# genlm/genlm-backend

Hardware: AMD Instinct MI355X
Metric: particles/sec + logprob-kernel HBM GB/s (% of 8 TB/s), 1024 particles gpt2 (higher is better)
Workload: dtype f32

## Files before the change

### genlm-backend_amd/_lib.py

```python
import ctypes as C
import os

_HERE = os.path.dirname(os.path.abspath(__file__))
LIB_PATH = os.path.join(_HERE, "libglb_hip.so")

ABI_VERSION = 9
GLB_OK, GLB_EINVAL, GLB_EUNSUPPORTED, GLB_EHIP, GLB_ENOSPC = 0, 1, 2, 3, 4
F32, BF16, F16 = 0, 1, 2
MASK_NONE, MASK_BITS, MASK_F32, MASK_PREPARED = 0, 1, 2, 3
RNG_NONE, RNG_PHILOX, RNG_NOISE = 0, 1, 2
STEP_HW_EXP = 1
GEMM_BIAS, GEMM_BIAS_GELU_TANH = 0, 1
GEMM_FORM_LARGE, GEMM_FORM_SMALL = 1, 2


class GlbError(RuntimeError):
    def __init__(self, code, msg):
        super().__init__(f"glb error {code}: {msg}")
        self.code = code


class StepArgs(C.Structure):
    _fields_ = [
        ("struct_size", C.c_uint32),
# ... 310 lines not shown
class FsaProductArgs(C.Structure):
    _fields_ = [
        ("struct_size", C.c_uint32),
        ("op", C.c_int32),
        ("n_a", C.c_int32), ("n_b", C.c_int32), ("start_a", C.c_int32), ("start_b", C.c_int32),
        ("delta_a", C.c_void_p), ("delta_b", C.c_void_p),
        ("accepting_a", C.c_void_p), ("accepting_b", C.c_void_p),
        ("live_a", C.c_void_p), ("live_b", C.c_void_p),
        ("arc_a", C.c_void_p), ("final_a", C.c_void_p),
        ("arc_b", C.c_void_p), ("final_b", C.c_void_p),
        ("max_states", C.c_int32),
        ("n_states", C.c_int32),
        ("table", C.c_void_p), ("table_slots", C.c_int64),
        ("pairs", C.c_void_p), ("delta_out", C.c_void_p), ("accepting_out", C.c_void_p),
        ("arc_out", C.c_void_p), ("final_out", C.c_void_p),
        ("live", C.c_void_p), ("counts", C.c_void_p), ("status", C.c_void_p),
        ("rounds", C.c_int32), ("restart", C.c_int32),
    ]


NFA_STATUS = 16
NFA_CLOSURE_STATUS = 8
NFA_MAX_IMPORTANT = 4096
NFA_MAX_STATES = 1 << 22


class NfaArgs(C.Structure):
    _fields_ = [
        ("struct_size", C.c_uint32),
        ("n_states", C.c_int32), ("start", C.c_int32),
        ("n_important", C.c_int32), ("n_words", C.c_int32),
        ("n_arcs", C.c_int32), ("n_eps", C.c_int32), ("n_groups", C.c_int32),
        ("eps_off", C.c_void_p), ("eps_to", C.c_void_p), ("bit_of", C.c_void_p),
        ("arc_off", C.c_void_p), ("arc_dst", C.c_void_p), ("arc_bytes", C.c_void_p), ("accepting_mask", C.c_void_p),
        ("group_of", C.c_void_p), ("group_lo", C.c_void_p),
        ("eclose", C.c_void_p),
        ("hash_mask", C.c_uint64),
        ("max_states", C.c_int32), ("chunk", C.c_int32),
        ("table", C.c_void_p), ("table_slots", C.c_int64),
        ("cand", C.c_void_p), ("sets", C.c_void_p),
        ("delta_out", C.c_void_p), ("accepting_out", C.c_void_p), ("counts", C.c_void_p), ("status", C.c_void_p),
        ("rounds", C.c_int32), ("restart", C.c_int32),
    ]


LAZY_STATUS = 8
LAZY_OVERFLOW, LAZY_BUG = 1, 2


class LazyArgs(C.Structure):
    _fields_ = [
        ("struct_size", C.c_uint32),
        ("dfa", DfaArgs),
        ("n_nfa_states", C.c_int32), ("nfa_start", C.c_int32),
        ("n_important", C.c_int32), ("n_words", C.c_int32),
        ("n_arcs", C.c_int32),
        ("max_states", C.c_int32),
        ("arc_off", C.c_void_p), ("arc_dst", C.c_void_p), ("arc_bytes", C.c_void_p), ("accepting_mask", C.c_void_p),
        ("eclose", C.c_void_p),
        ("hash_mask", C.c_uint64),
        ("table", C.c_void_p), ("table_slots", C.c_int64),
        ("cand", C.c_void_p), ("counts", C.c_void_p), ("cand_rows", C.c_int64),
        ("sets", C.c_void_p), ("accepting_out", C.c_void_p), ("status", C.c_void_p),
        ("row_state", C.c_void_p), ("row_stamp", C.c_void_p), ("claimants", C.c_void_p), ("victims", C.c_void_p),
        ("ecounters", C.c_void_p), ("epoch", C.c_void_p),
        ("force_wave", C.c_int32),
    ]


PDA_MAX_DEPTH = 504
PDA_STATUS = 8
PDA_OVERFLOW, PDA_BUG = 1, 2
PDA_MAX_SYMBOLS, PDA_POP = 126, 127


class PdaArgs(C.Structure):
    _fields_ = [
        ("struct_size", C.c_uint32),
        ("dfa", DfaArgs),
        ("n_pda_states", C.c_int32), ("n_symbols", C.c_int32), ("start", C.c_int32),
        ("max_depth", C.c_int32), ("n_words", C.c_int32), ("max_states", C.c_int32),
        ("delta", C.c_void_p), ("accepting", C.c_void_p),
        ("hash_mask", C.c_uint64),
        ("table", C.c_void_p), ("table_slots", C.c_int64),
        ("cand", C.c_void_p), ("counts", C.c_void_p), ("cand_rows", C.c_int64),
        ("configs", C.c_void_p), ("accepting_out", C.c_void_p), ("status", C.c_void_p),
        ("row_state", C.c_void_p), ("row_stamp", C.c_void_p), ("claimants", C.c_void_p), ("victims", C.c_void_p),
        ("ecounters", C.c_void_p), ("epoch", C.c_void_p),
        ("max_token_bytes", C.c_int32),
    ]


CONJ_MAX_PARTS = 8
CONJ_STATUS = 8
CONJ_OVERFLOW, CONJ_BUG = 1, 2


class ConjArgs(C.Structure):
    _fields_ = [
        ("struct_size", C.c_uint32),
        ("dfa", DfaArgs),
        ("n_parts", C.c_int32), ("n_words", C.c_int32), ("max_states", C.c_int32),
        ("part_start", C.c_int32 * CONJ_MAX_PARTS),
        ("hash_mask", C.c_uint64),
        ("table", C.c_void_p), ("table_slots", C.c_int64),
        ("tuples", C.c_void_p), ("status", C.c_void_p),
        ("counts", C.c_void_p), ("cand_rows", C.c_int64),
        ("part_states", C.c_void_p), ("part_ld", C.c_int64),
        ("claim_states", C.c_void_p), ("rep", C.c_void_p),
        ("part_rows", C.c_void_p * CONJ_MAX_PARTS), ("part_bank", C.c_void_p * CONJ_MAX_PARTS),
        ("part_bank_ld", C.c_int64 * CONJ_MAX_PARTS), ("part_capacity", C.c_int64 * CONJ_MAX_PARTS),
        ("part_weighted", C.c_int32 * CONJ_MAX_PARTS),
        ("wbank", C.c_void_p), ("wbank_ld", C.c_int64),
        ("row_state", C.c_void_p), ("row_stamp", C.c_void_p), ("claimants", C.c_void_p), ("victims", C.c_void_p),
        ("ecounters", C.c_void_p), ("epoch", C.c_void_p),
    ]


class ImportanceArgs(C.Structure):
    _fields_ = [
        ("struct_size", C.c_uint32),
        ("target", C.c_void_p), ("target_dtype", C.c_int32), ("ld_p", C.c_int64),
        ("proposal", C.c_void_p), ("proposal_dtype", C.c_int32), ("ld_q", C.c_int64),
        ("n_rows", C.c_int64), ("vocab", C.c_int64),
        ("proposal_scale", C.c_float),
        ("n_particles", C.c_int64), ("row_of", C.c_void_p),
        ("mask_kind", C.c_int32), ("mask", C.c_void_p), ("mask_ld", C.c_int64), ("n_masks", C.c_int64),
        ("mask_id", C.c_void_p), ("row_mask_id", C.c_void_p),
        ("seed", C.c_uint64), ("offset", C.c_uint64), ("particle_base", C.c_int64),
        ("out_token", C.c_void_p), ("out_dlogw", C.c_void_p), ("out_lse_target", C.c_void_p),
        ("out_logZ_proposal", C.c_void_p),
        ("workspace", C.c_void_p), ("workspace_bytes", C.c_size_t),
    ]


IMPORTANCE_CHUNK = 4096
IMPORTANCE_RECORD_BYTES = 64


class ScoreArgs(C.Structure):
    _fields_ = [
        ("struct_size", C.c_uint32),
        ("logits", C.c_void_p), ("dtype", C.c_int32),
        ("n_rows", C.c_int64), ("vocab", C.c_int64), ("ld", C.c_int64),
        ("logit_scale", C.c_float),
        ("token", C.c_void_p),
        ("mask_kind", C.c_int32), ("mask", C.c_void_p), ("mask_ld", C.c_int64), ("n_masks", C.c_int64),
        ("row_mask_id", C.c_void_p),
        ("out_logp", C.c_void_p), ("out_lse", C.c_void_p), ("out_logZ", C.c_void_p), ("out_logp_masked", C.c_void_p),
        ("seq_start", C.c_void_p), ("n_seq", C.c_int64),
        ("out_seq_logp", C.c_void_p), ("out_seq_logZ", C.c_void_p), ("out_seq_logp_masked", C.c_void_p),
    ]


_vp, _i32, _i64, _f32, _sz = C.c_void_p, C.c_int32, C.c_int64, C.c_float, C.c_size_t
SYMBOLS = {
    "glb_version": (C.c_char_p, []),
    "glb_abi_version": (C.c_int, []),
    "glb_last_error": (C.c_int, [C.c_char_p, _sz]),
    "glb_device_count": (C.c_int, []),
    "glb_step_workspace_bytes": (_sz, [_i64, _i64, _i64, _i64]),
    "glb_logprob_mask_sample": (C.c_int, [C.POINTER(StepArgs), _vp]),
    "glb_logprob_mask_sample_timed": (C.c_int, [C.POINTER(StepArgs), _vp, _vp, _vp]),
    "glb_workspace_init": (C.c_int, [_vp, _sz, _vp]),
    "glb_workspace_release": (C.c_int, [_vp]),
    "glb_workspace_check": (C.c_int, [_vp, _vp]),
    "glb_workspace_error_word": (_vp, [_vp]),
    "glb_set_spin_limit": (C.c_int, [C.c_uint64]),
    "glb_mask_prepared_bytes": (_sz, [_i64, _i64]),
    "glb_mask_prepare": (C.c_int, [_vp, _i64, _i64, _i64, _i32, _vp, _sz, _vp]),
    "glb_mask_prepare_rows": (C.c_int, [_vp, _i64, _i64, _i64, _i32, _vp, _i64, _vp, _sz, _vp]),
    "glb_log_softmax_workspace_bytes": (_sz, [_i64, _i64]),
    "glb_log_softmax_rows": (C.c_int, [_vp, _i32, _i64, _i64, _i64, _f32, _vp, _i32, _i64, _vp, _vp, _sz, _vp]),
    "glb_mask_f32_to_bits": (C.c_int, [_vp, _i64, _i64, _i64, _vp, _i64, _vp, _vp]),
    "glb_group_contexts_workspace": (_sz, [_i64]),
    "glb_group_contexts": (C.c_int, [_vp, _vp, _vp, _i64, _vp, _vp, _vp, _vp, _vp, _sz, _vp]),
    "glb_hash_contexts": (C.c_int, [_vp, _vp, _vp, _i64, _vp, _vp]),
    "glb_match_prefixes": (C.c_int, [_vp, _vp, _vp, _i64, _vp, _vp, _vp, _i64, _vp, _vp, _vp]),
    "glb_gather_padded": (C.c_int, [_vp, _vp, _vp, _vp, _i64, _vp, _i64, _i64, _i64, _vp, _vp, _vp, _vp, _vp]),
    "glb_gather_kv_padded": (C.c_int, [_vp, _vp, _i64, _vp, _i64, _i64, _i64, _i64, _i32, _vp, _vp]),
    "glb_particles_advance": (C.c_int, [_vp, _i64, _vp, _vp, _vp, _vp, _vp, _i64, _i32, _i32, _vp, _vp]),
    "glb_normalize_weights": (C.c_int, [_vp, _i64, _vp, _vp, _vp]),
    "glb_kv_append": (C.c_int, [_vp, _vp, _vp, _vp, _i64, _i64, _i64, _i64, _i64, _i64, _i32, _vp]),
    "glb_kv_gather_rows": (C.c_int, [_vp, _vp, _i64, _i64, _i64, _i64, _i64, _i64, _vp, _vp, _i32, _vp]),
    "glb_gather_rows_i32": (C.c_int, [_vp, _i64, _vp, _i64, _i64, _vp, _i64, _vp]),
    "glb_match_rows": (C.c_int, [_vp, _vp, _vp, _vp, _vp, _i64, _vp, _vp, _vp, _i64, _i64, _vp, _vp, _vp]),
    "glb_slab_attention": (C.c_int, [_vp, _i64, _i64, _vp, _i64, _i64, _vp, _i64, _i64, _vp, _vp, _vp, _i64, _i64, _i64, _i64, _i64,
                                     _f32, _i32, _vp, _vp]),
    "glb_short_attention": (C.c_int, [_vp, C.POINTER(C.c_int64), _vp, C.POINTER(C.c_int64), _vp, C.POINTER(C.c_int64), _vp, _i64, _i64,
                                      _i64, _i64, _i64, _i64, _i64, _i64, _f32, _i32, _vp, _vp]),
    "glb_short_attention_packed": (C.c_int, [_vp, _i64, _i64, _vp, _i64, _i64, _vp, _i64, _i64, _vp, _i64, _i64, _i64, _i64, _i64,
                                             _i64, _f32, _i32, _vp, _vp, _vp]),
    "glb_kv_plan_workspace": (_sz, [_i64, _i64]),
    "glb_kv_plan": (C.c_int, [C.POINTER(KvPlanArgs), _vp]),
    "glb_match_prefix_rows": (C.c_int, [_vp, _vp, _vp, _vp, _vp, _i64, _vp, _vp, _vp, _i64, _i64, _i32, _vp, _vp, _vp, _vp]),
    "glb_kv_plan_chunk": (C.c_int, [C.POINTER(KvPlanChunkArgs), _vp]),
    "glb_slab_attention_chunk": (C.c_int, [_vp, C.POINTER(C.c_int64), _vp, C.POINTER(C.c_int64), _vp, C.POINTER(C.c_int64), _vp, _vp,
                                           _vp, _vp, _vp, _i64, _i64, _i64, _i64, _i64, _i64, _i64, _f32, _i32, _vp, _vp]),
    "glb_trie_workspace": (_sz, [_i64, _i64]),
    "glb_trie_reduce": (C.c_int, [_vp, _i64, _i64, _i64, _i64, _i64, _vp, _vp, _vp, _vp, _vp, _i32, _i32, _vp, _i64, _vp, _sz,
                                  _vp]),
    "glb_trie_workspace_ex": (_sz, [_i64, _i64]),
    "glb_trie_masses": (C.c_int, [C.POINTER(TrieArgs), _vp]),
    "glb_trie_rows_workspace": (_sz, [_i64, C.POINTER(TriePlan)]),
    "glb_trie_rows": (C.c_int, [C.POINTER(TrieRowsArgs), C.POINTER(TriePlan), _vp]),
    "glb_resample_workspace": (_sz, [_i64]),
    "glb_resample_systematic": (C.c_int, [_vp, _i64, C.c_uint64, C.c_uint64, _vp, _vp, _vp, _sz, _vp]),
    "glb_mt19937_seed": (None, [C.POINTER(MT19937), C.c_uint64]),
    "glb_mt19937_exponential_f32": (C.c_int, [C.POINTER(MT19937), _vp, _i64]),
    "glb_mt19937_window": (C.c_int, [C.c_uint64, _vp]),
    "glb_mt19937_jump_polys": (C.c_int, [_i64, _i32, _i32, _vp]),
    "glb_mt19937_jump_host": (C.c_int, [_vp, _vp, _vp]),
    "glb_mt19937_rows_workspace": (_sz, [_i64, _i32]),
    "glb_mt19937_exponential_rows": (C.c_int, [C.POINTER(MtRowsArgs), _vp]),
    "glb_comm_unique_id": (C.c_int, [_vp]),
    "glb_comm_init": (C.c_int, [_vp, _i32, _i32, C.POINTER(C.c_void_p)]),
    "glb_allgather_f32": (C.c_int, [_vp, _vp, _i64, _vp, _vp]),
    "glb_comm_destroy": (C.c_int, [_vp]),
    "glb_gemm_split_bytes": (_sz, [_i64, _i64]),
    "glb_gemm_split_weights": (C.c_int, [_vp, _i64, _i64, _i64, _vp, _sz, _vp]),
    "glb_gemm_f32_split": (C.c_int, [C.POINTER(GemmArgs), _vp]),
    "glb_gemm_split_pick": (C.c_int, [_i64, _i64, _i64, C.c_int, C.POINTER(C.c_int)]),
    "glb_gemm_f32_split_form": (C.c_int, [C.POINTER(GemmArgs), C.c_int, _vp]),
    "glb_gemm_split_blocks_per_cu": (C.c_int, [C.c_int, C.POINTER(C.c_int)]),
    "glb_gemm_split_form_blocks_per_cu": (C.c_int, [C.c_int, C.c_int, C.POINTER(C.c_int)]),
    "glb_lora_merge_workspace_bytes": (_sz, [_i32]),
    "glb_lora_merge": (C.c_int, [C.POINTER(LoraJob), _i32, _vp, _sz, _vp]),
    "glb_lora_rows_table_bytes": (_sz, [_i32, _i32]),
    "glb_lora_rows_table_upload": (C.c_int, [C.POINTER(LoraRowsEntry), _i32, _i32, _vp, _sz, _vp]),
    "glb_lora_rows_workspace_bytes": (_sz, [_i64, _i32]),
    "glb_lora_rows": (C.c_int, [C.POINTER(LoraRowsArgs), _vp]),
    "glb_w4_bytes": (_sz, [_i64, _i64]),
    "glb_w4_quantize": (C.c_int, [C.POINTER(W4Args), _vp]),
    "glb_w4_dequantize": (C.c_int, [C.POINTER(W4Args), _vp]),
    "glb_w4_gemm_max_rows": (C.c_int, []),
    "glb_w4_gemm_workspace_bytes": (_sz, [_i64, _i64, _i64]),
    "glb_w4_gemm": (C.c_int, [C.POINTER(W4GemmArgs), _vp]),
    "glb_dfa_bank_init": (C.c_int, [C.POINTER(DfaArgs), _vp]),
    "glb_dfa_advance": (C.c_int, [C.POINTER(DfaArgs), _vp]),
    "glb_dfa_claim_rows": (C.c_int, [C.POINTER(DfaArgs), _vp]),
    "glb_dfa_fill_masks": (C.c_int, [C.POINTER(DfaArgs), _vp]),
    "glb_dfa_mask_ids": (C.c_int, [C.POINTER(DfaArgs), _vp]),
    "glb_dfa_bank_rows": (_i64, [_sz, _i64, _i64]),
    "glb_dfa_weight_bank_init": (C.c_int, [C.POINTER(DfaWeightArgs), _vp]),
    "glb_dfa_fill_weights": (C.c_int, [C.POINTER(DfaWeightArgs), _vp]),
    "glb_dfa_weight_bank_rows": (_i64, [_sz, _i64, _i64]),
    "glb_dfa_evict_bank_init": (C.c_int, [C.POINTER(DfaEvictArgs), _vp]),
    "glb_dfa_evict_serve": (C.c_int, [C.POINTER(DfaEvictArgs), _vp]),
    "glb_dfa_backward": (C.c_int, [C.POINTER(DfaPushArgs), _vp]),
    "glb_dfa_push_weights": (C.c_int, [C.POINTER(DfaPushArgs), _vp]),
    "glb_dfa_refine": (C.c_int, [C.POINTER(DfaMinArgs), _vp]),
    "glb_dfa_quotient": (C.c_int, [C.POINTER(DfaMinArgs), _vp]),
    "glb_fsa_product_round": (C.c_int, [C.POINTER(FsaProductArgs), _vp]),
    "glb_fsa_live": (C.c_int, [C.POINTER(FsaProductArgs), _vp]),
    "glb_nfa_closure": (C.c_int, [C.POINTER(NfaArgs), _vp]),
    "glb_nfa_subset_round": (C.c_int, [C.POINTER(NfaArgs), _vp]),
    "glb_lazy_init": (C.c_int, [C.POINTER(LazyArgs), _vp]),
    "glb_lazy_advance": (C.c_int, [C.POINTER(LazyArgs), _vp]),
    "glb_lazy_serve": (C.c_int, [C.POINTER(LazyArgs), _vp]),
    "glb_pda_init": (C.c_int, [C.POINTER(PdaArgs), _vp]),
    "glb_pda_advance": (C.c_int, [C.POINTER(PdaArgs), _vp]),
    "glb_pda_serve": (C.c_int, [C.POINTER(PdaArgs), _vp]),
    "glb_conj_init": (C.c_int, [C.POINTER(ConjArgs), _vp]),
    "glb_conj_unpack": (C.c_int, [C.POINTER(ConjArgs), _vp]),
    "glb_conj_number": (C.c_int, [C.POINTER(ConjArgs), _vp]),
    "glb_conj_serve": (C.c_int, [C.POINTER(ConjArgs), _vp]),
    "glb_importance_workspace_bytes": (_sz, [_i64, _i64, _i64]),
    "glb_importance_step": (C.c_int, [C.POINTER(ImportanceArgs), _vp]),
    "glb_score_rows": (C.c_int, [C.POINTER(ScoreArgs), _vp]),
    "glb_score_seq_sums": (C.c_int, [_vp, _i64, _vp, _i64, _vp, _vp]),
    "glb_philox4x32_10": (None, [C.POINTER(C.c_uint32), C.POINTER(C.c_uint32), C.POINTER(C.c_uint32)]),
}

_lib = None


def load():
    global _lib
    if _lib is not None:
        return _lib
    if not os.path.exists(LIB_PATH):
        raise ImportError(
            f"{LIB_PATH} not found: build it with `make -C genlm-backend_amd/csrc -j8` "
            "(or `python -c 'import __graft_entry__ as g; g.build()'`). There is no CPU fallback."
        )
    import torch

    lib = C.CDLL(LIB_PATH)
    for name, (res, args) in SYMBOLS.items():
        fn = getattr(lib, name)
        fn.restype = res
        fn.argtypes = args
    if lib.glb_abi_version() != ABI_VERSION:
        raise ImportError(f"libglb_hip.so ABI {lib.glb_abi_version()} != {ABI_VERSION}")
    _lib = lib
    return lib


def last_error():
    buf = C.create_string_buffer(512)
    load().glb_last_error(buf, 512)
    return buf.value.decode()


def check(rc):
    if rc != GLB_OK:
        raise GlbError(rc, last_error())
```

### genlm-backend_amd/csrc/glb_api.hip

```cpp
#include <hip/hip_ext.h>
#include <hip/hip_runtime.h>

#include <atomic>
#include <cmath>
#include <cstdarg>
#include <cstdio>
#include <cstdlib>
#include <cstring>
#include <mutex>
#include <string>
#include <unordered_map>

#include "../../include/glb.h"
#include "glb_chunk.hpp"
#include "glb_common.hpp"

namespace glb {
#define GLB_DECL(dt)                                                                                              \
  hipError_t launch_stats_##dt(const StepParams &p, int mask_kind, bool scaled, int expc, hipStream_t s);          \
  hipError_t launch_fused_step_##dt(const StepParams &p, int mask_kind, int mode, bool scaled, int expc,          \
                                    hipStream_t s);                                                               \
  hipError_t launch_finish_##dt(const StepParams &p, int mask_kind, int mode, int expc, hipStream_t s);           \
  hipError_t launch_logprob_rows_##dt(const void *logits, int64_t ld, int V, float scale, const float *lse,       \
                                      void *out, bool out16, int64_t out_ld, int n_rows, hipStream_t s);           \
// ... 371 lines not shown
        const int64_t si0 = (int64_t)(((uint64_t)s0h << 32) | s0l);
        const bool like = i < n && h[k] == (((uint64_t)h0h << 32) | h0l) && li[k] == l0 &&
                          (si[k] == si0 || same_tokens(tok + si[k], tok + si0, li[k]));
        all_same = __ballot(like) == act;
      }
    }
    if (i < n && (!all_same || lane == leader)) {
      int32_t s = (int32_t)(h[k] & (uint64_t)(cap - 1));
      for (;;) {
        const int32_t owner = atomicCAS(&s_table[s], -1, i);
        if (owner == -1 || owner == i) break;
        if constexpr (HASHED) {
          if (hash_in[owner] == h[k] && len[owner] == li[k] && same_tokens(tok + si[k], tok + st[owner], li[k])) break;
        } else {
          if (s_hash[owner] == h[k] && s_len[owner] == li[k] && same_tokens(tok + si[k], tok + s_st[owner], li[k])) break;
        }
        s = (s + 1) & (cap - 1);
      }
      slot[k] = s;
      atomicMin(&s_min[s], i);
    }
    if (all_same) slot[k] = __builtin_amdgcn_readlane(slot[k], leader);
  }
  __syncthreads();
  int32_t flag[PER], mine = 0;
#pragma unroll
  for (int k = 0; k < PER; ++k) {
    const int i = tid * PER + k;
    flag[k] = (i < n && s_min[slot[k]] == i) ? 1 : 0;
    mine += flag[k];
  }
  int32_t incl = mine;
#pragma unroll
  for (int o = 1; o < 64; o <<= 1) {
    const int32_t t = __shfl_up(incl, o, 64);
    if (lane >= o) incl += t;
  }
  if (lane == 63) s_wave[wave] = incl;
  __syncthreads();
  int32_t g = incl - mine, total = 0;
#pragma unroll
  for (int w = 0; w < 16; ++w) {
    const int32_t v = s_wave[w];
    if (w < wave) g += v;
    total += v;
  }
#pragma unroll
  for (int k = 0; k < PER; ++k) {
    if (flag[k]) {
      s_table[slot[k]] = g;
      out_rep[g] = tid * PER + k;
      ++g;
    }
  }
  if (tid == 0) *out_n_groups = total;
  __syncthreads();
#pragma unroll
  for (int k = 0; k < PER; ++k) {
    const int i = tid * PER + k;
    if (i < n) out_group_of[i] = s_table[slot[k]];
  }
}

__global__ void match_prefixes_kernel(const int32_t *tok, const int64_t *st, const int32_t *len,
                                      int64_t n, const int32_t *ptok, const int64_t *pst,
                                      const int32_t *plen, int64_t np, int32_t *out_prefix,
                                      int32_t *out_base) {
  const int64_t i = (int64_t)blockIdx.x * blockDim.x + threadIdx.x;
  if (i >= n) return;
  const int64_t li = len[i];
  const int32_t *c = tok + st[i];
  int32_t best = -1;
  int64_t bl = 0;
  for (int64_t k = 0; k < np; ++k) {
    const int64_t lk = plen[k];
    if (lk >= li || lk <= bl) continue;
    const int32_t *q = ptok + pst[k];
    bool eq = true;
    for (int64_t t = 0; t < lk; ++t)
      if (q[t] != c[t]) {
        eq = false;
        break;
      }
    if (eq) {
      best = (int32_t)k;
      bl = lk;
    }
  }
  out_prefix[i] = best;
  out_base[i] = (int32_t)bl;
}

__global__ void gather_padded_kernel(const int32_t *tok, const int64_t *st, const int32_t *lens,
                                     const int32_t *sel, int64_t n_sel, const int32_t *base, int64_t pad_id,
                                     int64_t p_max, int64_t l_max, int64_t *ids, int64_t *am,
                                     int64_t *pos, int32_t *last) {
  const int64_t width = p_max + l_max;
  const int64_t gid = (int64_t)blockIdx.x * blockDim.x + threadIdx.x;
  if (gid >= n_sel * width) return;
  const int64_t u = gid / width, p = gid % width;
  const int64_t s = sel ? sel[u] : u;
  const int64_t b = base ? base[s] : 0;
  int64_t len = (int64_t)lens[s] - b;
  len = len < 0 ? 0 : (len > l_max ? l_max : len);
  if (p < p_max) {
    am[gid] = p < b ? 1 : 0;
  } else {
    const int64_t t = p - p_max;
    const bool in = t < len;
    am[gid] = in ? 1 : 0;
    ids[u * l_max + t] = in ? (int64_t)tok[st[s] + b + t] : pad_id;
    pos[u * l_max + t] = in ? b + t : 0;
    if (t == 0 && last) last[u] = (int32_t)(len - 1);
  }
}

template <typename VT>
__global__ void gather_kv_kernel(const void *const *slabs, const int32_t *slab_len,
                                 const int32_t *prefix_of, int64_t n_rows, int64_t heads,
                                 int64_t row_vecs, int64_t p_max, VT *out) {
  const int64_t gid = (int64_t)blockIdx.x * blockDim.x + threadIdx.x;
  const int64_t total = n_rows * heads * p_max * row_vecs;
  if (gid >= total) return;
  const int64_t x = gid % row_vecs;
  const int64_t pp = (gid / row_vecs) % p_max;
  const int64_t h = (gid / (row_vecs * p_max)) % heads;
  const int64_t u = gid / (row_vecs * p_max * heads);
  const int32_t k = prefix_of[u];
  VT v{};
  if (k >= 0) {
    const int64_t pl = slab_len[k];
    if (pp < pl) v = reinterpret_cast<const VT *>(slabs[k])[(h * pl + pp) * row_vecs + x];
  }
  out[gid] = v;
}

__global__ void particles_advance_kernel(int32_t *ctx, int64_t ctx_ld, int32_t *len,
                                         int32_t *active, float *lw, const float *logZ,
                                         const int32_t *tok, int64_t n, int32_t eos,
                                         int32_t max_len, uint64_t *hashes) {
  const int64_t i = (int64_t)blockIdx.x * blockDim.x + threadIdx.x;
  if (i >= n || !active[i]) return;
  const int32_t t = tok[i];
  if (t == -2) return;
  lw[i] += logZ[i];
  if (t == eos || t < 0) {
    active[i] = 0;
  } else {
    const int32_t l = len[i];
    ctx[i * ctx_ld + l] = t;
    len[i] = l + 1;
    if (hashes) hashes[i] = ctx_hash_step(hashes[i], (uint32_t)t);
    if (l + 1 >= max_len) active[i] = 0;
  }
}

}

extern "C" {

const char *glb_version(void) { return "glb-hip 0.2.0 (gfx950)"; }
int glb_abi_version(void) { return GLB_ABI_VERSION; }

int glb_last_error(char *buf, size_t n) {
  if (!buf || n == 0) return GLB_EINVAL;
  snprintf(buf, n, "%s", g_err.c_str());
  return GLB_OK;
}

int glb_device_count(void) {
  int c = 0;
  if (hipGetDeviceCount(&c) != hipSuccess) {
    (void)hipGetLastError();
    return -1;
  }
  return c;
}

size_t glb_step_workspace_bytes(int64_t n_particles, int64_t n_rows, int64_t vocab, int64_t n_masks) {
  if (n_particles <= 0 || vocab <= 0) return 0;
  const int64_t units = n_particles > n_rows ? n_particles : n_rows;
  return step_fixed_bytes(units, vocab) + (n_masks > 0 ? prepared_bytes(n_masks, vocab) : 0) + 256;
}

size_t glb_mask_prepared_bytes(int64_t n_masks, int64_t vocab) {
  if (n_masks <= 0 || vocab <= 0) return 0;
  return prepared_bytes(n_masks, vocab);
}

int glb_mask_prepare(const uint32_t *mask_bits, int64_t n_masks, int64_t vocab, int64_t mask_ld, int32_t dtype,
                     void *out_prepared, size_t out_bytes, void *stream) {
  if (!mask_bits || !out_prepared) return fail(GLB_EINVAL, "null pointer");
  if (n_masks <= 0 || vocab <= 0 || mask_ld < (vocab + 31) / 32) return fail(GLB_EINVAL, "bad sizes");
  if (dtype < GLB_F32 || dtype > GLB_F16) return fail(GLB_EINVAL, "bad dtype %d", dtype);
  if (vocab > 0x7fffff00ll || n_masks > 65535) return fail(GLB_EINVAL, "vocab / n_masks out of range");
  if (out_bytes < prepared_bytes(n_masks, vocab))
    return fail(GLB_ENOSPC, "prepared buffer %zu < %zu bytes", out_bytes, prepared_bytes(n_masks, vocab));
  if (((uintptr_t)out_prepared) % 16 || ((uintptr_t)mask_bits) % 4) return fail(GLB_EINVAL, "misaligned pointer");
  const hipError_t e = launch_mask_prepare(mask_bits, n_masks, vocab, mask_ld, dtype, out_prepared, (hipStream_t)stream);
  if (e != hipSuccess) return hip_fail(e, "mask_prepare launch");
  return GLB_OK;
}

int glb_mask_prepare_rows(const uint32_t *mask_bits, int64_t n_masks, int64_t vocab, int64_t mask_ld, int32_t dtype,
                          const int32_t *rows, int64_t n_rows, void *prepared, size_t prepared_bytes_, void *stream) {
  if (!mask_bits || !prepared || (n_rows > 0 && !rows)) return fail(GLB_EINVAL, "null pointer");
  if (n_masks <= 0 || vocab <= 0 || mask_ld < (vocab + 31) / 32 || n_rows < 0) return fail(GLB_EINVAL, "bad sizes");
  if (dtype < GLB_F32 || dtype > GLB_F16) return fail(GLB_EINVAL, "bad dtype %d", dtype);
  if (vocab > 0x7fffff00ll || n_masks > 65535 || n_rows > 65535) return fail(GLB_EINVAL, "vocab / n_masks / n_rows out of range");
  if (prepared_bytes_ < prepared_bytes(n_masks, vocab))
    return fail(GLB_ENOSPC, "prepared buffer %zu < %zu bytes", prepared_bytes_, prepared_bytes(n_masks, vocab));
  if (((uintptr_t)prepared) % 16 || ((uintptr_t)mask_bits) % 4) return fail(GLB_EINVAL, "misaligned pointer");
  if (n_rows == 0) return GLB_OK;
  const hipError_t e = launch_mask_prepare(mask_bits, n_masks, vocab, mask_ld, dtype, prepared, (hipStream_t)stream, nullptr, rows, n_rows);
  if (e != hipSuccess) return hip_fail(e, "mask_prepare launch");
  return GLB_OK;
}

int glb_logprob_mask_sample(const glb_step_args *a, void *stream) {
  if (!a) return fail(GLB_EINVAL, "glb_logprob_mask_sample: null args");
  if (a->struct_size != sizeof(glb_step_args))
    return fail(GLB_EINVAL, "glb_step_args.struct_size %u != %zu (ABI mismatch)", a->struct_size,
                sizeof(glb_step_args));
  if (!a->logits) return fail(GLB_EINVAL, "logits is null");
  if (a->dtype < GLB_F32 || a->dtype > GLB_F16) return fail(GLB_EINVAL, "bad dtype %d", a->dtype);
  if (a->n_rows <= 0 || a->vocab <= 0 || a->n_particles <= 0)
    return fail(GLB_EINVAL, "n_rows=%lld vocab=%lld n_particles=%lld must be positive",
                (long long)a->n_rows, (long long)a->vocab, (long long)a->n_particles);
  if (a->ld < a->vocab) return fail(GLB_EINVAL, "ld %lld < vocab %lld", (long long)a->ld, (long long)a->vocab);
  if (a->vocab > 0x7fffff00ll || a->n_particles > 0x7fffffffll || a->n_rows > 0x7fffffffll)
    return fail(GLB_EINVAL, "vocab / n_particles / n_rows exceed 31 bits");
  const int es = a->dtype == GLB_F32 ? 4 : 2;
  if (((uintptr_t)a->logits) % es) return fail(GLB_EINVAL, "logits pointer not element aligned");
  if (!a->row_of && a->n_particles != a->n_rows)
    return fail(GLB_EINVAL, "row_of is null but n_particles != n_rows");
  if (a->mask_kind < GLB_MASK_NONE || a->mask_kind > GLB_MASK_PREPARED)
    return fail(GLB_EINVAL, "bad mask_kind %d", a->mask_kind);
  const bool by_row = a->mask_kind == GLB_MASK_NONE || a->row_mask_id != nullptr;
  const int64_t n_units = by_row ? a->n_rows : a->n_particles;
  if (a->mask_kind != GLB_MASK_NONE) {
    if (!a->mask || a->n_masks <= 0) return fail(GLB_EINVAL, "mask table missing");
    if (a->mask_kind != GLB_MASK_PREPARED) {
      const int64_t need = a->mask_kind == GLB_MASK_BITS ? (a->vocab + 31) / 32 : a->vocab;
      if (a->mask_ld < need) return fail(GLB_EINVAL, "mask_ld %lld < %lld", (long long)a->mask_ld, (long long)need);
    }
    if (a->row_mask_id && a->mask_id) return fail(GLB_EINVAL, "give mask_id (per particle) or row_mask_id (per row), not both");
    if (!a->row_mask_id && !a->mask_id && a->n_masks != 1 && a->n_masks != n_units)
      return fail(GLB_EINVAL, "no mask ids given but n_masks is neither 1 nor the number of %s",
                  by_row ? "rows" : "particles");
    if (((uintptr_t)a->mask) % (a->mask_kind == GLB_MASK_PREPARED ? 16 : 4)) return fail(GLB_EINVAL, "mask pointer misaligned");
    if (a->n_masks > 0x7fffffffll) return fail(GLB_EINVAL, "n_masks exceeds 31 bits");
  }
  if (a->rng_mode < GLB_RNG_NONE || a->rng_mode > GLB_RNG_NOISE)
    return fail(GLB_EINVAL, "bad rng_mode %d", a->rng_mode);
  if (a->flags & ~GLB_STEP_HW_EXP) return fail(GLB_EINVAL, "flags %d: only GLB_STEP_HW_EXP is defined", a->flags);
  const int expc = (a->flags & GLB_STEP_HW_EXP) ? glb::kExpHw : glb::kExpPoly;
  if (a->rng_mode == GLB_RNG_NOISE && (!a->noise || (a->noise_ld < a->vocab && a->noise_ld != 0)))
    return fail(GLB_EINVAL, "noise tensor missing or noise_ld < vocab (0 = one row shared by every particle)");
  if (a->rng_mode != GLB_RNG_NONE && !a->out_token)
    return fail(GLB_EINVAL, "rng_mode set but out_token is null");
  if (!(a->logit_scale == a->logit_scale)) return fail(GLB_EINVAL, "logit_scale is NaN");
  if (!a->workspace) return fail(GLB_EINVAL, "workspace is null (glb_step_workspace_bytes)");
  if (((uintptr_t)a->workspace) % 32) return fail(GLB_EINVAL, "workspace not 32-byte aligned");
  const bool own_prep = a->mask_kind == GLB_MASK_BITS;
  const size_t fixed_bytes = step_fixed_bytes(n_units, a->vocab);
  const size_t need_ws = fixed_bytes + (own_prep ? prepared_bytes(a->n_masks, a->vocab) : 0);
  if (a->workspace_bytes < need_ws)
    return fail(GLB_ENOSPC, "workspace %zu < %zu bytes", a->workspace_bytes, need_ws);

  hipStream_t s = (hipStream_t)stream;
  glb::StepParams p{};
  p.logits = a->logits;
  p.ld = a->ld;
  p.V = (int32_t)a->vocab;
  p.nch = (int32_t)n_chunks(a->vocab);
  p.scale = a->logit_scale;
  p.n_particles = (int32_t)a->n_particles;
  p.n_pairs = (int32_t)n_units;
  p.n_masks = (int32_t)a->n_masks;
  if (by_row) {
    p.pair_row = nullptr;
    p.pair_mask = a->row_mask_id;
    p.pair_of = a->row_of;
  } else {
    p.pair_row = a->row_of;
    p.pair_mask = a->mask_id;
    p.pair_of = nullptr;
  }
  p.recs = (uint64_t *)a->workspace;
  p.noise = a->noise;
  p.noise_ld = a->noise_ld;
  p.seed = a->seed;
  p.offset = a->offset;
  p.particle_base = a->particle_base;
  p.out_logZ = a->out_logZ;
  p.out_lse = a->out_lse;
  p.out_token = a->out_token;
#ifdef GLB_STAMPS
  p.out_margin = a->out_margin;
#else
  p.out_margin = a->rng_mode == GLB_RNG_NOISE ? a->out_margin : nullptr;
#endif
  const bool scaled = a->logit_scale != 1.0f;
  const int64_t items = n_units * (int64_t)p.nch;
  const bool fmask = a->mask_kind == GLB_MASK_F32;
  bool fused = a->rng_mode != GLB_RNG_NOISE && items > 512 && a->n_particles <= 16 * (int64_t)fin_wave_cap(fmask);
// ... 211 lines not shown
size_t glb_group_contexts_workspace(int64_t n) {
  if (n <= 0) return 0;
  return (size_t)(2 * group_cap(n) + 2 * n) * sizeof(int32_t) + (size_t)n * sizeof(uint64_t) + 8;
}

int glb_hash_contexts(const int32_t *tokens, const int64_t *starts, const int32_t *lengths, int64_t n,
                      uint64_t *out_hashes, void *stream) {
  if (!tokens || !starts || !lengths || !out_hashes) return fail(GLB_EINVAL, "null pointer");
  if (n <= 0 || n > (1 << 28)) return fail(GLB_EINVAL, "n out of range");
  hipLaunchKernelGGL(hash_contexts_kernel, dim3(blocks_for(n, 64)), dim3(64), 0, (hipStream_t)stream, tokens, starts,
                     lengths, (int32_t)n, out_hashes);
  const hipError_t e = hipGetLastError();
  if (e != hipSuccess) return hip_fail(e, "hash_contexts launch");
  return GLB_OK;
}

int glb_group_contexts(const int32_t *tokens, const int64_t *starts, const int32_t *lengths,
                       int64_t n, const uint64_t *ctx_hashes, int32_t *out_group_of, int32_t *out_rep,
                       int32_t *out_n_groups, void *workspace, size_t workspace_bytes, void *stream) {
  if (!tokens || !starts || !lengths || !out_group_of || !out_rep || !out_n_groups || !workspace)
    return fail(GLB_EINVAL, "null pointer");
  if (n <= 0 || n > (1 << 28)) return fail(GLB_EINVAL, "n out of range");
  if (workspace_bytes < glb_group_contexts_workspace(n))
    return fail(GLB_ENOSPC, "workspace %zu < %zu bytes", workspace_bytes, glb_group_contexts_workspace(n));
  const int64_t cap = group_cap(n);
  if (n <= 8192) {
    const size_t lds = (size_t)cap * 2 * sizeof(int32_t);
    hipStream_t s = (hipStream_t)stream;
    if (n < 256 && !ctx_hashes) {
      const size_t lds1 = lds + 1024 * (sizeof(uint64_t) + sizeof(int64_t) + sizeof(int32_t));
      hipLaunchKernelGGL((group_contexts_lds_kernel<1, false>), dim3(1), dim3(1024), lds1, s, tokens, starts, lengths,
                         (int32_t)n, (int32_t)cap, out_group_of, out_rep, out_n_groups, (const uint64_t *)nullptr);
    } else {
      const uint64_t *hashes = ctx_hashes;
      if (!hashes) {
        uint64_t *hw = (uint64_t *)((char *)workspace + (size_t)(2 * cap + 2 * n) * sizeof(int32_t));
        hipLaunchKernelGGL(hash_contexts_kernel, dim3(blocks_for(n, 64)), dim3(64), 0, s, tokens, starts, lengths,
                           (int32_t)n, hw);
        hashes = hw;
      }
      if (n <= 1024) {
        hipLaunchKernelGGL((group_contexts_lds_kernel<1, true>), dim3(1), dim3(1024), lds, s, tokens, starts, lengths,
                           (int32_t)n, (int32_t)cap, out_group_of, out_rep, out_n_groups, hashes);
      } else if (n > 4096) {
        static std::atomic<uint64_t> big_lds{0};
        const hipError_t big_lds_rc = glb::allow_dynamic_lds((const void *)group_contexts_lds_kernel<8, true>, 128 * 1024, big_lds);
        if (big_lds_rc != hipSuccess) return hip_fail(big_lds_rc, "hipFuncSetAttribute(group_contexts)");
        hipLaunchKernelGGL((group_contexts_lds_kernel<8, true>), dim3(1), dim3(1024), lds, s, tokens, starts, lengths,
                           (int32_t)n, (int32_t)cap, out_group_of, out_rep, out_n_groups, hashes);
      } else if (n <= 2048) {
        hipLaunchKernelGGL((group_contexts_lds_kernel<2, true>), dim3(1), dim3(1024), lds, s, tokens, starts, lengths,
                           (int32_t)n, (int32_t)cap, out_group_of, out_rep, out_n_groups, hashes);
      } else {
        hipLaunchKernelGGL((group_contexts_lds_kernel<4, true>), dim3(1), dim3(1024), lds, s, tokens, starts, lengths,
                           (int32_t)n, (int32_t)cap, out_group_of, out_rep, out_n_groups, hashes);
      }
    }
    const hipError_t e = hipGetLastError();
    if (e != hipSuccess) return hip_fail(e, "group_contexts launch");
    return GLB_OK;
  }
  int32_t *table = (int32_t *)workspace, *minidx = table + cap, *slot_of = minidx + cap, *gid_of = slot_of + n;
  const uint64_t *hashes = ctx_hashes;
  hipStream_t s = (hipStream_t)stream;
  hipLaunchKernelGGL(group_init_kernel, dim3(blocks_for(cap, 256)), dim3(256), 0, s, (int32_t)cap, table, minidx);
  if (!hashes) {
    uint64_t *hw = (uint64_t *)(gid_of + n);
    hipLaunchKernelGGL(hash_contexts_kernel, dim3(blocks_for(n, 256)), dim3(256), 0, s, tokens, starts, lengths, (int32_t)n,
                       hw);
    hashes = hw;
  }
  hipLaunchKernelGGL(group_insert_kernel, dim3(blocks_for(n, 256)), dim3(256), 0, s, tokens, starts, lengths, (int32_t)n,
                     (int32_t)cap, hashes, table, minidx, slot_of);
  hipLaunchKernelGGL(group_number_kernel, dim3(1), dim3(1024), 0, s, (int32_t)n, minidx, slot_of, gid_of, out_group_of,
                     out_rep, out_n_groups);
  const hipError_t e = hipGetLastError();
  if (e != hipSuccess) return hip_fail(e, "group_contexts launch");
  return GLB_OK;
}

int glb_match_prefixes(const int32_t *tokens, const int64_t *starts, const int32_t *lengths,
                       int64_t n, const int32_t *prefix_tokens, const int64_t *prefix_starts,
                       const int32_t *prefix_lengths, int64_t n_prefixes, int32_t *out_prefix,
                       int32_t *out_base, void *stream) {
  if (!tokens || !starts || !lengths || !out_prefix || !out_base) return fail(GLB_EINVAL, "null pointer");
  if (n <= 0 || n_prefixes < 0) return fail(GLB_EINVAL, "bad sizes");
  if (n_prefixes > 0 && (!prefix_tokens || !prefix_starts || !prefix_lengths))
    return fail(GLB_EINVAL, "null prefix table");
  hipLaunchKernelGGL(match_prefixes_kernel, dim3(blocks_for(n, 256)), dim3(256), 0,
                     (hipStream_t)stream, tokens, starts, lengths, n, prefix_tokens, prefix_starts,
                     prefix_lengths, n_prefixes, out_prefix, out_base);
  const hipError_t e = hipGetLastError();
  if (e != hipSuccess) return hip_fail(e, "match_prefixes launch");
  return GLB_OK;
}

int glb_gather_padded(const int32_t *tokens, const int64_t *starts, const int32_t *lengths,
                      const int32_t *sel, int64_t n_sel, const int32_t *base, int64_t pad_id, int64_t p_max,
                      int64_t l_max, int64_t *out_input_ids, int64_t *out_attention_mask,
                      int64_t *out_position_ids, int32_t *out_last_index, void *stream) {
  if (!tokens || !starts || !lengths || !out_input_ids || !out_attention_mask || !out_position_ids)
    return fail(GLB_EINVAL, "null pointer");
  if (n_sel <= 0 || l_max <= 0 || p_max < 0) return fail(GLB_EINVAL, "bad sizes");
  const int64_t total = n_sel * (p_max + l_max);
  hipLaunchKernelGGL(gather_padded_kernel, dim3(blocks_for(total, 256)), dim3(256), 0,
                     (hipStream_t)stream, tokens, starts, lengths, sel, n_sel, base, pad_id, p_max, l_max,
                     out_input_ids, out_attention_mask, out_position_ids, out_last_index);
  const hipError_t e = hipGetLastError();
  if (e != hipSuccess) return hip_fail(e, "gather_padded launch");
  return GLB_OK;
}

int glb_gather_kv_padded(const void *const *slabs, const int32_t *slab_len, int64_t n_prefixes,
                         const int32_t *prefix_of, int64_t n_rows, int64_t heads, int64_t head_dim,
                         int64_t p_max, int32_t elem_bytes, void *out, void *stream) {
  if (!slabs || !slab_len || !prefix_of || !out) return fail(GLB_EINVAL, "null pointer");
  if (n_prefixes <= 0 || n_rows <= 0 || heads <= 0 || head_dim <= 0 || p_max <= 0)
    return fail(GLB_EINVAL, "bad sizes");
  if (elem_bytes != 2 && elem_bytes != 4) return fail(GLB_EINVAL, "elem_bytes must be 2 or 4");
  const int64_t rowb = head_dim * elem_bytes;
  hipStream_t s = (hipStream_t)stream;
  if (rowb % 16 == 0 && ((uintptr_t)out) % 16 == 0) {
    const int64_t rv = rowb / 16, total = n_rows * heads * p_max * rv;
    hipLaunchKernelGGL(gather_kv_kernel<uint4>, dim3(blocks_for(total, 256)), dim3(256), 0, s,
                       slabs, slab_len, prefix_of, n_rows, heads, rv, p_max, (uint4 *)out);
  } else if (elem_bytes == 4) {
    const int64_t total = n_rows * heads * p_max * head_dim;
    hipLaunchKernelGGL(gather_kv_kernel<uint32_t>, dim3(blocks_for(total, 256)), dim3(256), 0, s,
                       slabs, slab_len, prefix_of, n_rows, heads, head_dim, p_max, (uint32_t *)out);
  } else {
    const int64_t total = n_rows * heads * p_max * head_dim;
    hipLaunchKernelGGL(gather_kv_kernel<uint16_t>, dim3(blocks_for(total, 256)), dim3(256), 0, s,
                       slabs, slab_len, prefix_of, n_rows, heads, head_dim, p_max, (uint16_t *)out);
  }
  const hipError_t e = hipGetLastError();
  if (e != hipSuccess) return hip_fail(e, "gather_kv launch");
  return GLB_OK;
}

int glb_particles_advance(int32_t *contexts, int64_t ctx_ld, int32_t *lengths, int32_t *active,
                          float *log_weights, const float *logZ, const int32_t *token, int64_t n,
                          int32_t eos_id, int32_t max_len, uint64_t *hashes, void *stream) {
  if (!contexts || !lengths || !active || !log_weights || !logZ || !token)
    return fail(GLB_EINVAL, "null pointer");
  if (n <= 0 || ctx_ld <= 0 || max_len > ctx_ld) return fail(GLB_EINVAL, "bad sizes");
  hipLaunchKernelGGL(particles_advance_kernel, dim3(blocks_for(n, 256)), dim3(256), 0,
                     (hipStream_t)stream, contexts, ctx_ld, lengths, active, log_weights, logZ,
                     token, n, eos_id, max_len, hashes);
  const hipError_t e = hipGetLastError();
  if (e != hipSuccess) return hip_fail(e, "particles_advance launch");
  return GLB_OK;
}

void glb_philox4x32_10(const uint32_t ctr[4], const uint32_t key[2], uint32_t out[4]) {
  glb::philox4x32_10(ctr, key, out);
}

}
```

### genlm-backend_amd/engine.py

```python
import ctypes as C

import numpy as np
import torch

from . import _lib
from ._lib import GLB_EHIP, GlbError
from ._lib import (F32, BF16, F16, MASK_NONE, MASK_BITS, MASK_F32, MASK_PREPARED, RNG_NONE, RNG_PHILOX, RNG_NOISE,
                   STEP_HW_EXP, KvPlanArgs, KvPlanChunkArgs, MtRowsArgs, StepArgs, TrieArgs, TriePlan, TrieRowsArgs, MT19937, MT_POLY_WORDS, check)

_DT = {torch.float32: F32, torch.bfloat16: BF16, torch.float16: F16}


def _ptr(t):
    return None if t is None else C.c_void_p(t.data_ptr())


class LoraRowsTable:

    def __init__(self, dev, n_slots, n_modules, r_max, keep):
        self.dev, self.n_slots, self.n_modules, self.r_max, self.keep = dev, n_slots, n_modules, r_max, keep


class HostRng:

    def __init__(self, seed):
        self._lib = _lib.load()
        self.state = MT19937()
        self._lib.glb_mt19937_seed(C.byref(self.state), C.c_uint64(seed))

    def exponential(self, n, out=None):
        if out is None:
            out = torch.empty(n, dtype=torch.float32, pin_memory=torch.cuda.is_available())
        assert out.dtype == torch.float32 and out.is_contiguous() and out.device.type == "cpu"
        check(self._lib.glb_mt19937_exponential_f32(C.byref(self.state), _ptr(out), n))
        return out


def _low_priority_stream(device):
    try:
        hip = C.CDLL("libamdhip64.so")
        least, greatest = C.c_int(0), C.c_int(0)
        if hip.hipDeviceGetStreamPriorityRange(C.byref(least), C.byref(greatest)) == 0 and least.value > 0:
            h = C.c_void_p()
            with torch.cuda.device(device):
                if hip.hipStreamCreateWithPriority(C.byref(h), C.c_uint(1), C.c_int(least.value)) == 0 and h.value:
                    return torch.cuda.ExternalStream(h.value, device=device)
    except OSError:
        pass
    return torch.cuda.Stream(device=device)


class DeviceRng:

    SMALL = 32

    def __init__(self, engine, seed, vocab, ahead=False):
        self.eng, self.seed, self.vocab, self.ahead = engine, int(seed), int(vocab), bool(ahead)
        self._side = None
        self._pre = None
        self._ws = None
        self._last = None
        self.reset()

    def reset(self):
        if self._pre is not None:
            self._pre[2].synchronize()
            self._pre = None
        w = np.zeros(624, np.uint32)
        check(self.eng.lib.glb_mt19937_window(C.c_uint64(self.seed & 0xFFFFFFFFFFFFFFFF), C.c_void_p(w.ctypes.data)))
        self.window = torch.from_numpy(w.view(np.int32)).to(self.eng.device)
        self.rows_drawn = 0

    def _args(self, max_draw, n_big, polys):
        eng = self.eng
        need = eng.lib.glb_mt19937_rows_workspace(max_draw, self.SMALL)
        if self._ws is None or self._ws.numel() < need:
            self._ws = torch.empty(need, dtype=torch.uint8, device=eng.device)
        a = MtRowsArgs()
        a.struct_size = C.sizeof(MtRowsArgs)
        a.window = self.window.data_ptr()
        a.polys = polys.data_ptr()
        a.n_small, a.n_big = self.SMALL, n_big
        a.vocab, a.max_draw_rows = self.vocab, max_draw
        a.workspace, a.workspace_bytes = self._ws.data_ptr(), self._ws.numel()
        return a

    def rows(self, n_out, row_slot=None, n_draw=None, max_draw=None, out=None):
        eng, V = self.eng, self.vocab
        max_draw = int(n_out if max_draw is None else max_draw)
        polys, n_big = eng.mt_polys(V, max_draw + 1)
        if out is None:
            out = torch.empty((n_out, V), dtype=torch.float32, device=eng.device)
        eng._check_dev(row_slot, n_draw, out)
        if row_slot is not None and (row_slot.dtype != torch.int32 or row_slot.numel() != n_out):
            raise ValueError("row_slot must be int32 [n_out]")
        if n_draw is not None and n_draw.dtype != torch.int32:
            raise TypeError("n_draw must be an int32 device scalar")
        pre, self._pre = self._pre, None
        if pre is not None and pre[0] != max_draw:
            pre[2].synchronize()
            pre = None
        a = self._args(max_draw, n_big, polys)
        a.window_out = self.window.data_ptr()
        a.n_draw = None if n_draw is None else n_draw.data_ptr()
        a.n_out_rows = n_out
        a.row_slot = None if row_slot is None else row_slot.data_ptr()
        a.out, a.out_ld = out.data_ptr(), out.stride(0) if n_out > 1 else max(V, out.stride(0))
        if pre is not None:
            torch.cuda.current_stream(eng.device).wait_event(pre[2])
            a.reuse_windows = 1
            a.rows_from, a.rows_from_ld = pre[1].data_ptr(), pre[1].stride(0)
        check(eng.lib.glb_mt19937_exponential_rows(C.byref(a), eng._stream()))
        if n_draw is None:
            self.rows_drawn += max_draw
        self._last = max_draw
        return out

    def prefetch(self):
        if not self.ahead or self._last is None or self._pre is not None:
            return
        eng, V, max_draw = self.eng, self.vocab, self._last
        if self._side is None:
            self._side = _low_priority_stream(eng.device)
            self._rows_buf = None
        if self._rows_buf is None or self._rows_buf.shape[0] < max_draw:
            self._rows_buf = torch.empty((max_draw, V), dtype=torch.float32, device=eng.device)
        polys, n_big = eng.mt_polys(V, max_draw + 1)
        a = self._args(max_draw, n_big, polys)
        a.n_out_rows = max_draw
        a.out, a.out_ld = self._rows_buf.data_ptr(), self._rows_buf.stride(0)
        self._side.wait_stream(torch.cuda.current_stream(eng.device))
        with torch.cuda.stream(self._side):
            check(eng.lib.glb_mt19937_exponential_rows(C.byref(a), eng._stream()))
            done = torch.cuda.Event()
            done.record(self._side)
        self._pre = (max_draw, self._rows_buf, done)


class PreparedMasks:

    def __init__(self, blob, n_masks, vocab, dtype):
        self.blob, self.n_masks, self.vocab, self.dtype = blob, n_masks, vocab, dtype


class StepPlan:

    __slots__ = ("eng", "args", "keep", "out", "_ref")

    def __init__(self, eng, args, keep, out):
        self.eng, self.args, self.keep, self.out = eng, args, keep, out
        self._ref = C.byref(args)

    def run(self, offset=None, seed=None):
        a = self.args
        if offset is not None:
            a.offset = offset
        if seed is not None:
            a.seed = seed
        if self.eng._step_ws is not self.keep[-1]:
            raise RuntimeError("the engine's scratch buffer was reallocated since this plan was made: make a new plan")
        check(self.eng.lib.glb_logprob_mask_sample(self._ref, self.eng._stream()))
        return self.out

    def run_timed(self, events, offset=None, seed=None):
        a = self.args
        if offset is not None:
            a.offset = offset
# ... 284 lines not shown
            setattr(a, "out_" + w, out[w].data_ptr())
        if seq_start is not None:
            if seq_start.dtype != torch.int64 or seq_start.dim() != 1 or seq_start.numel() < 1 or not seq_start.is_contiguous():
                raise ValueError("seq_start must be a contiguous int64 [n_seq + 1] tensor")
            a.seq_start, a.n_seq = seq_start.data_ptr(), seq_start.numel() - 1
            for w in want:
                if w != "lse":
                    out["seq_" + w] = self._f32(a.n_seq)
                    setattr(a, "out_seq_" + w, out["seq_" + w].data_ptr())
        check(self.lib.glb_score_rows(C.byref(a), self._stream()))
        return out

    def score_seq_sums(self, values, seq_start):
        self._check_dev(values, seq_start)
        if values.dtype != torch.float32 or values.dim() != 1:
            raise ValueError("values must be a float32 [n_rows] tensor")
        if seq_start.dtype != torch.int64 or seq_start.dim() != 1 or seq_start.numel() < 1:
            raise ValueError("seq_start must be an int64 [n_seq + 1] tensor")
        out = self._f32(seq_start.numel() - 1)
        if out.numel():
            src = values if values.numel() else out
            check(self.lib.glb_score_seq_sums(_ptr(src), values.numel(), _ptr(seq_start), out.numel(), _ptr(out), self._stream()))
        return out

    def error_word(self):
        ws = self._step_ws
        if ws is None:
            return torch.zeros(1, dtype=torch.int32, device=self.device)
        return ws[ws.numel() - 64: ws.numel() - 60].view(torch.int32)

    def raise_if_failed(self, err_count=None, tokens=None, lse=None, what="glb_logprob_mask_sample"):
        bad = bool(err_count)
        if tokens is not None and not bad:
            bad = bool((np.asarray(tokens) == -2).any())
        if lse is not None and not bad:
            bad = bool(np.isnan(np.asarray(lse, dtype=np.float32)).any())
        if bad:
            if self._step_ws is not None:
                self.error_word().zero_()
            raise GlbError(GLB_EHIP, f"{what}: waves of the launch gave up waiting for their row's records (token -2 / "
                                     "NaN): the call did not complete and its results must not be used")

    def check(self):
        if self._step_ws is not None:
            check(self.lib.glb_workspace_check(_ptr(self._step_ws), self._stream()))

    def set_spin_limit(self, microseconds):
        check(self.lib.glb_set_spin_limit(0xFFFFFFFFFFFFFFFF if microseconds is None else int(microseconds)))

    def timing_events(self, n):
        with torch.cuda.device(self.device):
            pairs = [(torch.cuda.Event(enable_timing=True), torch.cuda.Event(enable_timing=True)) for _ in range(n)]
            for a, b in pairs:
                a.record()
                b.record()
            torch.cuda.current_stream(self.device).synchronize()
        return pairs

    def step_plan(self, logits, **kw):
        return self.step(logits, _plan=True, **kw)

    def noise_rng(self, seed, vocab, ahead=False):
        return DeviceRng(self, seed, vocab, ahead=ahead)

    def mt_polys(self, vocab, n_windows):
        small = DeviceRng.SMALL
        need_big = max(1, -(-int(n_windows) // small))
        ent = self._mt_polys.get(vocab)
        if ent is None or ent[1] < need_big:
            n_big = max(need_big, 2 * ent[1] if ent else 0)
            host = np.zeros((small + n_big, MT_POLY_WORDS), np.uint64)
            check(self.lib.glb_mt19937_jump_polys(2 * int(vocab), small, n_big, C.c_void_p(host.ctypes.data)))
            ent = self._mt_polys[vocab] = (torch.from_numpy(host.view(np.int64)).to(self.device), n_big)
        return ent

    def prepare_masks(self, bits, vocab, logits_dtype=torch.float32):
        if bits.dim() == 1:
            bits = bits[None]
        self._check_dev(bits)
        if bits.dtype != torch.int32:
            raise TypeError("bit masks must be int32 words")
        K = bits.shape[0]
        need = self.lib.glb_mask_prepared_bytes(K, vocab)
        blob = torch.empty(need, dtype=torch.uint8, device=self.device)
        dt = _DT[logits_dtype]
        check(self.lib.glb_mask_prepare(_ptr(bits), K, vocab, bits.stride(0) if K > 1 else bits.shape[1], dt,
                                        _ptr(blob), need, self._stream()))
        return PreparedMasks(blob, K, vocab, dt)

    def update_prepared_masks(self, prepared, bits, rows):
        if bits.dim() == 1:
            bits = bits[None]
        self._check_dev(bits, rows)
        if bits.dtype != torch.int32 or rows.dtype != torch.int32:
            raise TypeError("bit masks and row indices must be int32")
        if bits.shape[0] != prepared.n_masks:
            raise ValueError("the bit rows are not the ones these masks were prepared from")
        K = prepared.n_masks
        check(self.lib.glb_mask_prepare_rows(_ptr(bits), K, prepared.vocab, bits.stride(0) if K > 1 else bits.shape[1], prepared.dtype,
                                             _ptr(rows), rows.numel(), _ptr(prepared.blob), prepared.blob.numel(), self._stream()))
        return prepared

    def log_softmax_rows(self, logits, vocab=None, logit_scale=1.0, out=None, want_lse=False, workspace=None,
                         out_dtype=torch.float32):
        if logits.dim() != 2 or logits.stride(1) != 1:
            raise ValueError("logits must be 2-D with unit inner stride")
        n_rows, width = logits.shape
        V = width if vocab is None else vocab
        ld = logits.stride(0) if n_rows > 1 else max(width, logits.stride(0))
        if out is None:
            out = torch.empty((n_rows, V), dtype=out_dtype, device=self.device)
        if out.dtype not in (torch.float32, logits.dtype):
            raise TypeError(f"log-probabilities leave as float32 or as {logits.dtype}, not {out.dtype}")
        lse = self._f32(n_rows) if want_lse else None
        out_ld = out.stride(0) if n_rows > 1 else max(V, out.stride(0))
        need = self.lib.glb_log_softmax_workspace_bytes(n_rows, V)
        ws = self._scratch(need) if workspace is None else workspace
        if ws.numel() < need:
            raise ValueError(f"workspace of {ws.numel()} bytes, {need} needed")
        check(self.lib.glb_log_softmax_rows(_ptr(logits), _DT[logits.dtype], n_rows, V, ld, logit_scale, _ptr(out),
                                            _DT[out.dtype], out_ld, _ptr(lse), _ptr(ws), ws.numel(), self._stream()))
        return (out, lse) if want_lse else out

    def row_lse(self, logits, vocab=None, logit_scale=1.0):
        if logits.dim() != 2 or logits.stride(1) != 1:
            raise ValueError("logits must be 2-D with unit inner stride")
        n_rows, width = logits.shape
        V = width if vocab is None else vocab
        ld = logits.stride(0) if n_rows > 1 else max(width, logits.stride(0))
        lse = self._f32(n_rows)
        ws = self._scratch(self.lib.glb_log_softmax_workspace_bytes(n_rows, V))
        check(self.lib.glb_log_softmax_rows(_ptr(logits), _DT[logits.dtype], n_rows, V, ld, logit_scale, None, F32, 0,
                                            _ptr(lse), _ptr(ws), ws.numel(), self._stream()))
        return lse

    def mask_to_bits(self, mask):
        if mask.dim() == 1:
            mask = mask[None]
        mask = mask.to(self.device, torch.float32).contiguous()
        K, V = mask.shape
        W = (V + 31) // 32
        bits = torch.empty((K, W), dtype=torch.int32, device=self.device)
        flag = self._i32(1)
        check(self.lib.glb_mask_f32_to_bits(_ptr(mask), K, V, V, _ptr(bits), W, _ptr(flag), self._stream()))
        return bits, flag

    def hash_contexts(self, tokens, starts, lengths):
        n = lengths.numel()
        self._check_dev(tokens, starts, lengths)
        out = torch.empty(n, dtype=torch.int64, device=self.device)
        check(self.lib.glb_hash_contexts(_ptr(tokens), _ptr(starts), _ptr(lengths), n, _ptr(out), self._stream()))
        return out

    def group_contexts(self, tokens, starts, lengths, hashes=None):
        n = lengths.numel()
        self._check_dev(tokens, starts, lengths, hashes)
        need = self.lib.glb_group_contexts_workspace(n)
        if self._ws is None or self._ws.numel() < need:
            self._ws = torch.empty(max(need, 1 << 16), dtype=torch.uint8, device=self.device)
        group_of, rep, ng = self._i32(n), self._i32(n), self._i32(1)
        check(self.lib.glb_group_contexts(_ptr(tokens), _ptr(starts), _ptr(lengths), n, _ptr(hashes), _ptr(group_of),
                                          _ptr(rep), _ptr(ng), _ptr(self._ws), self._ws.numel(), self._stream()))
        return group_of, rep, ng

    def match_prefixes(self, tokens, starts, lengths, prefix_tokens, prefix_starts, prefix_lengths):
        n = lengths.numel()
        npre = 0 if prefix_lengths is None else prefix_lengths.numel()
        pref, base = self._i32(n), self._i32(n)
        check(self.lib.glb_match_prefixes(_ptr(tokens), _ptr(starts), _ptr(lengths), n, _ptr(prefix_tokens),
                                          _ptr(prefix_starts), _ptr(prefix_lengths), npre, _ptr(pref), _ptr(base),
                                          self._stream()))
        return pref, base

    def gather_padded(self, tokens, starts, lengths, sel, n_sel, base, pad_id, p_max, l_max):
        dev = self.device
        ids = torch.empty((n_sel, l_max), dtype=torch.int64, device=dev)
        am = torch.empty((n_sel, p_max + l_max), dtype=torch.int64, device=dev)
        pos = torch.empty((n_sel, l_max), dtype=torch.int64, device=dev)
        last = self._i32(n_sel)
        check(self.lib.glb_gather_padded(_ptr(tokens), _ptr(starts), _ptr(lengths), _ptr(sel), n_sel, _ptr(base),
                                         pad_id, p_max, l_max, _ptr(ids), _ptr(am), _ptr(pos), _ptr(last),
                                         self._stream()))
        return ids, am, pos, last

    def gather_kv_padded(self, slab_ptrs, slab_len, prefix_of, heads, head_dim, p_max, dtype):
        n_rows = prefix_of.numel()
        out = torch.empty((n_rows, heads, p_max, head_dim), dtype=dtype, device=self.device)
        check(self.lib.glb_gather_kv_padded(_ptr(slab_ptrs), _ptr(slab_len), slab_len.numel(), _ptr(prefix_of),
                                            n_rows, heads, head_dim, p_max, out.element_size(), _ptr(out),
                                            self._stream()))
        return out

    def particles_advance(self, contexts, lengths, active, log_weights, logZ, token, eos_id, max_len, hashes=None):
        n, ld = contexts.shape
        check(self.lib.glb_particles_advance(_ptr(contexts), ld, _ptr(lengths), _ptr(active), _ptr(log_weights),
                                             _ptr(logZ), _ptr(token), n, eos_id, max_len, _ptr(hashes), self._stream()))

    def normalize_weights(self, log_weights):
        n = log_weights.numel()
        probs, stats = self._f32(n), self._f32(2)
        check(self.lib.glb_normalize_weights(_ptr(log_weights), n, _ptr(probs), _ptr(stats), self._stream()))
        return probs, stats

    def gemm_split_supports(self, k, n):
        return self.lib.glb_gemm_split_bytes(k, n) > 0

    def gemm_split_blocks_per_cu(self, gelu=False, form=None):
        blocks = C.c_int(0)
        with torch.cuda.device(self.device):
            if form is None:
                check(self.lib.glb_gemm_split_blocks_per_cu(int(bool(gelu)), C.byref(blocks)))
            else:
                check(self.lib.glb_gemm_split_form_blocks_per_cu(int(form), int(bool(gelu)), C.byref(blocks)))
        return blocks.value

    def gemm_split_pick(self, m, n, k, n_cus=None):
        if n_cus is None:
            n_cus = torch.cuda.get_device_properties(self.device).multi_processor_count
        form = C.c_int(0)
        check(self.lib.glb_gemm_split_pick(m, n, k, n_cus, C.byref(form)))
        return form.value

    def gemm_split_weights(self, w):
        k, n = w.shape
        nbytes = self.lib.glb_gemm_split_bytes(k, n)
        if nbytes == 0 or w.dtype != torch.float32 or w.stride(1) != 1:
            return None
        if w.device != self.device:
            raise ValueError(f"tensor on {w.device}, engine on {self.device}")
        out =torch.empty(nbytes, dtype=torch.uint8, device=self.device)
        check(self.lib.glb_gemm_split_weights(_ptr(w), k, n, w.stride(0), _ptr(out), nbytes, self._stream()))
        return out

    def gemm_split(self, x, w_split, n, bias=None, gelu=False, out=None, form=None):
        k = x.shape[-1]
        x2 = x.reshape(-1, k)
        m = x2.shape[0]
        if m == 0 or x2.stride(1) != 1:
            return None
        if bias is not None:
            if bias.device != self.device:
                raise ValueError(f"bias on {bias.device}, engine on {self.device}")
            if bias.dim() != 1 or bias.numel() != n:
                raise ValueError(f"bias of shape {tuple(bias.shape)}, expected ({n},)")
            if bias.dtype != torch.float32 or bias.stride(0) != 1:
                return None
        if out is None:
            out = torch.empty((m, n), dtype=torch.float32, device=self.device)
        else:
            if out.device != self.device:
                raise ValueError(f"out on {out.device}, engine on {self.device}")
            if out.dtype != torch.float32 or tuple(out.shape) != (m, n):
                raise ValueError(f"out is {out.dtype} {tuple(out.shape)}, expected torch.float32 {(m, n)}")
            if out.stride(1) != 1 or (m > 1 and out.stride(0) < n):
                raise ValueError(f"out has strides {out.stride()}: rows of unit inner stride, at least {n} apart, are needed")
        a = _lib.GemmArgs()
        a.struct_size = C.sizeof(_lib.GemmArgs)
        a.m, a.n, a.k = m, n, k
        a.a, a.lda = x2.data_ptr(), x2.stride(0)
        a.w_split = w_split.data_ptr()
        a.bias = bias.data_ptr() if bias is not None else None
        a.c, a.ldc = out.data_ptr(), max(out.stride(0), n)
        a.epilogue = _lib.GEMM_BIAS_GELU_TANH if gelu else _lib.GEMM_BIAS
        if form is None:
            rc = self.lib.glb_gemm_f32_split(C.byref(a), self._stream())
        else:
            rc = self.lib.glb_gemm_f32_split_form(C.byref(a), int(form), self._stream())
        if rc == _lib.GLB_EUNSUPPORTED:
            return None
        check(rc)
        return out.view(*x.shape[:-1], n)

    def lora_merge(self, jobs):
        n = len(jobs)
        if n == 0:
            return
        table = (_lib.LoraJob * n)()
        for q, j in zip(table, jobs):
            w, a, b, out = j["w"], j["a"], j["b"], j["out"]
            for t in (w, a, b, out):
                if t.device != self.device:
                    raise ValueError(f"tensor on {t.device}, engine on {self.device}")
                if t.dim() != 2 or t.stride(1) != 1:
                    raise ValueError("lora_merge: every matrix must be 2-D with unit inner stride")
                if t.dtype not in _DT:
                    raise ValueError(f"lora_merge: unsupported dtype {t.dtype}")
            if a.dtype != b.dtype or out.dtype != w.dtype or out.shape != w.shape:
                raise ValueError("lora_merge: a / b must share a dtype, out must match w's dtype and shape")
            tr = bool(j.get("transposed", False))
            q.struct_size = C.sizeof(_lib.LoraJob)
            q.w_dtype, q.ab_dtype, q.w_transposed = _DT[w.dtype], _DT[a.dtype], int(tr)
            q.k_in, q.n_out = (w.shape[0], w.shape[1]) if tr else (w.shape[1], w.shape[0])
            q.r = a.shape[0]
            if tuple(a.shape) != (q.r, q.k_in) or tuple(b.shape) != (q.n_out, q.r):
                raise ValueError(f"lora_merge: a {tuple(a.shape)} / b {tuple(b.shape)} do not fit w {tuple(w.shape)}")
            q.w, q.ldw = w.data_ptr(), w.stride(0)
            q.a, q.lda = a.data_ptr(), a.stride(0)
            q.b, q.ldb = b.data_ptr(), b.stride(0)
            q.scale = float(j["scale"])
            q.out, q.ldo = out.data_ptr(), out.stride(0)
        nbytes = self.lib.glb_lora_merge_workspace_bytes(n)
        ws = torch.empty(nbytes, dtype=torch.uint8, device=self.device)
        check(self.lib.glb_lora_merge(table, n, _ptr(ws), nbytes, self._stream()))

    def lora_rows_table(self, slots):
        n_slots = len(slots)
        n_modules = len(slots[0]) if n_slots else 0
        nbytes = self.lib.glb_lora_rows_table_bytes(n_slots, n_modules)
        if nbytes == 0:
            raise ValueError(f"lora_rows_table: {n_slots} slots x {n_modules} modules is not served")
        host = (_lib.LoraRowsEntry * (n_slots * n_modules))()
        keep, r_max = [], 0
        for si, mods in enumerate(slots):
            if len(mods) != n_modules:
                raise ValueError("lora_rows_table: every slot lists every module")
            for mi, j in enumerate(mods):
                q = host[si * n_modules + mi]
                q.struct_size = C.sizeof(_lib.LoraRowsEntry)
                if j is None:
                    continue
                a, b = j["a"], j["b"]
                for t in (a, b):
                    if t.device != self.device:
                        raise ValueError(f"tensor on {t.device}, engine on {self.device}")
                    if t.dim() != 2 or t.stride(1) != 1 or t.dtype not in _DT:
                        raise ValueError("lora_rows_table: a / b must be 2-D float32 / bfloat16 / float16 with unit inner stride")
                if a.dtype != b.dtype or a.shape[0] != b.shape[1]:
                    raise ValueError("lora_rows_table: a / b must share a dtype and the rank")
                q.ab_dtype = _DT[a.dtype]
                q.n_out, q.k_in, q.r = b.shape[0], a.shape[1], a.shape[0]
                q.a, q.lda = a.data_ptr(), a.stride(0)
                q.b, q.ldb = b.data_ptr(), b.stride(0)
                q.scale = float(j["scale"])
                keep += [a, b]
                r_max = max(r_max, int(a.shape[0]))
        dev = torch.empty(nbytes, dtype=torch.uint8, device=self.device)
        check(self.lib.glb_lora_rows_table_upload(host, n_slots, n_modules, _ptr(dev), nbytes, self._stream()))
        return LoraRowsTable(dev, n_slots, n_modules, max(r_max, 1), keep)

    @staticmethod
    def _rows_2d(t, what):
        if t.dim() < 1 or t.stride(-1) != 1:
            raise ValueError(f"lora_rows: {what} must have unit inner stride")
        rows, pitch = 1, None
        for d in range(t.dim() - 2, -1, -1):
            if t.shape[d] == 1:
                continue
            if pitch is None:
                pitch = t.stride(d)
# ... 482 lines not shown
```

### genlm-backend_amd/kv.py

```python
import gc
import itertools
from collections import OrderedDict

import numpy as np
import torch
from transformers.cache_utils import Cache, CacheLayerMixin, DynamicCache


_ATTN_NAME = "glb"
SHORT_ATTENTION_MAX = 4096


def _glb_attention_forward(module, query, key, value, attention_mask, dropout=0.0, scaling=None, **kwargs):
    from transformers.integrations.sdpa_attention import sdpa_attention_forward

    layer = getattr(key, "_glb_layer", None)
    if layer is not None and layer._new_k is not None and getattr(layer.owner, "n_new", None) is not None:
        if key is not layer.keys or value is not layer.values:
            raise RuntimeError("glb_slab_attention_chunk: the attention module changed the key / value tensors the KV slab "
                               "handed out: the new tokens were never appended")
        k_new, v_new, layer._new_k, layer._new_v = layer._new_k, layer._new_v, None, None
        o = layer.owner
        scale = scaling if scaling is not None else query.shape[-1] ** -0.5
        return o.engine.slab_attention_chunk(query, k_new, v_new, layer.keys, layer.values, o.pos, o.n_new, scale, rows=o.rows), None
    if layer is not None and layer._new_k is not None:
        if key is not layer.keys or value is not layer.values or query.shape[2] != 1:
            raise RuntimeError("glb_slab_attention: the attention module changed the key / value tensors the KV slab handed "
                               "out (or feeds more than one token): the new token was never appended - run this model with "
                               "SlabForward(fused_attention=False)")
        k_new, v_new, layer._new_k, layer._new_v = layer._new_k, layer._new_v, None, None
        o = layer.owner
        scale = scaling if scaling is not None else query.shape[-1] ** -0.5
        return o.engine.slab_attention(query, k_new, v_new, layer.keys, layer.values, o.pos, scale), None
    packed = getattr(key, "_glb_packed", None)
    if packed is not None:
        if query.shape[0] != 1 or key.shape[2] != query.shape[2] or query.shape[2] != packed.n_rows or value.shape != key.shape:
            raise RuntimeError("glb_short_attention_packed: the attention module changed the shape of the packed batch")
        scale = scaling if scaling is not None else query.shape[-1] ** -0.5
        out = packed.engine.short_attention_packed(query[0].transpose(0, 1), key[0].transpose(0, 1), value[0].transpose(0, 1),
                                                   packed.segments, packed.max_keys, scale)
        packed.served += 1
        return out.unsqueeze(0), None
    eng = getattr(getattr(module, "config", None), "_glb_engine", None)
    Lq, Lk = query.shape[2], key.shape[2]
    wants_grad = torch.is_grad_enabled() and (query.requires_grad or key.requires_grad or value.requires_grad)
    if (eng is not None and query.is_cuda and not dropout and not wants_grad and not getattr(module, "training", False)
            and Lq * Lk <= SHORT_ATTENTION_MAX and Lk >= Lq
            and eng.slab_attention_supports(query.dtype, query.shape[-1]) and key.dtype == query.dtype == value.dtype
            and query.stride(3) == 1 and key.stride(3) == 1 and value.stride(3) == 1
            and kwargs.get("is_causal", True) is not False and not kwargs.get("softcap") and not kwargs.get("sliding_window")
            and getattr(module, "is_causal", True)
            and (attention_mask is None or (attention_mask.dtype == torch.bool and attention_mask.dim() == 4
                                            and attention_mask.shape[1] == 1 and attention_mask.shape[-1] == Lk
                                            and attention_mask.stride(3) == 1))
            and all((st * query.element_size()) % 16 == 0 for t in (query, key, value) for st in t.stride()[:3])
            and all(t.data_ptr() % 16 == 0 for t in (query, key, value))):
        scale = scaling if scaling is not None else query.shape[-1] ** -0.5
        return eng.short_attention(query, key, value, attention_mask, scale), None
    return sdpa_attention_forward(module, query, key, value, attention_mask, dropout=dropout, scaling=scaling, **kwargs)


def _register_attention():
    from transformers.masking_utils import ALL_MASK_ATTENTION_FUNCTIONS
    from transformers.modeling_utils import ALL_ATTENTION_FUNCTIONS

    if _ATTN_NAME not in ALL_ATTENTION_FUNCTIONS:
        ALL_ATTENTION_FUNCTIONS.register(_ATTN_NAME, _glb_attention_forward)
        ALL_MASK_ATTENTION_FUNCTIONS.register(_ATTN_NAME, ALL_MASK_ATTENTION_FUNCTIONS["sdpa"])


def use_glb_attention(shadow, engine):
    cfg = getattr(shadow, "config", None)
    if cfg is not None and getattr(cfg, "_attn_implementation", None) == _ATTN_NAME:
        return getattr(cfg, "_glb_engine", None) is engine
    if (cfg is None or not hasattr(engine, "short_attention") or getattr(cfg, "_attn_implementation", None) != "sdpa"
            or getattr(cfg, "attn_logit_softcapping", None) or getattr(cfg, "sliding_window", None)
            or getattr(cfg, "scale_attn_by_inverse_layer_idx", False)):
        return False
    _register_attention()
    cfg._attn_implementation = _ATTN_NAME
    cfg._glb_engine = engine
    return True


class _SlabLayer(CacheLayerMixin):

    is_compileable = False
    is_sliding = False

    def __init__(self, owner, idx):
        super().__init__()
        self.owner, self.idx = owner, idx
        self._new_k = self._new_v = None

    def lazy_initialization(self, key_states, value_states):
        o = self.owner
        shape_k = (o.n, key_states.shape[1], o.cap, key_states.shape[-1])
        shape_v = (o.n, value_states.shape[1], o.cap, value_states.shape[-1])
        self.keys = torch.zeros(shape_k, dtype=key_states.dtype, device=key_states.device)
        self.values = torch.zeros(shape_v, dtype=value_states.dtype, device=value_states.device)
        self.is_initialized = True

    def update(self, key_states, value_states, *args, **kwargs):
        if not self.is_initialized:
            self.lazy_initialization(key_states, value_states)
        o = self.owner
        if key_states.shape[0] != o.n or key_states.shape[-2] != 1:
            raise ValueError("SlabKV takes one new token for every particle per forward")
        if o.fused_attention:
            self._new_k, self._new_v = key_states, value_states
            self.keys._glb_layer = self
            return self.keys, self.values
        o.engine.kv_append(self.keys, key_states, o.pos)
        o.engine.kv_append(self.values, value_states, o.pos)
        return self.keys, self.values

    def get_mask_sizes(self, query_length):
        return self.owner.cap, 0

    def get_seq_length(self):
        return self.owner.cap - 1

    def get_max_length(self):
        return self.owner.cap


class SlabKV(Cache):
    def __init__(self, engine, n, cap, n_layers):
        self.engine, self.n, self.cap = engine, n, cap
        self.pos = None
        self.fused_attention = False
        super().__init__(layers=[_SlabLayer(self, i) for i in range(n_layers)])
        self._alt = None
        self._ptrs = None

    def set_forward_in_place(self, pos):
        self.pos = pos

    def attention_mask(self, pos):
        ar = torch.arange(self.cap, device=pos.device, dtype=pos.dtype)
        return (ar[None, :] <= pos[:, None]).to(torch.int64)

    def _alloc_like(self, prompt_layers):
        for layer, (k, v) in zip(self.layers, prompt_layers):
            if not layer.is_initialized:
                layer.lazy_initialization(k[:1], v[:1])

    def _tensors(self, which):
        return [t for layer in which for t in (layer.keys, layer.values)]

    def fill_rows(self, src_layers, src_row_of, len_of):
        self._alloc_like(src_layers)
        srcs = [t for kv in src_layers for t in kv]
        self.engine.kv_gather_rows(srcs, self._tensors(self.layers), src_row_of, len_of, srcs_stable=False)

    def gather(self, src_row_of, len_of):
        cur = self._tensors(self.layers)
        if self._alt is None:
            self._alt = [torch.zeros_like(t) for t in cur]
# ... 311 lines not shown
                src_full = torch.full((R + 1,), -1, dtype=torch.int32, device=dev)
                len_full = torch.zeros(R + 1, dtype=torch.int32, device=dev)
                src_full[slot] = torch.arange(nB, dtype=torch.int32, device=dev)
                len_full[slot] = batch[2][sel.long()]
                src_full[R] = -1
                self.pkv.fill_rows(srcs, src_full[:R].contiguous(), len_full[:R].contiguous())
        return (parts[0] if len(parts) == 1 else torch.cat(parts)), fed, in_place


def ragged(seqs):
    n = len(seqs)
    lens = np.fromiter(map(len, seqs), np.int32, n)
    starts = np.zeros(n, np.int64)
    starts[1:] = np.cumsum(lens[:-1])
    return np.fromiter(itertools.chain.from_iterable(seqs), np.int32, int(lens.sum())), starts, lens


class PrefixTable:

    def __init__(self, entries, device):
        self.kvs = kvs = [kv for kv, _ in entries]
        p0 = kvs[0]
        for p in kvs[1:]:
            if (p.heads, p.head_dim, p.dtype, len(p.layers)) != (p0.heads, p0.head_dim, p0.dtype, len(p0.layers)):
                raise ValueError("cached prefixes of different KV shapes in one batch")
        self.n = len(kvs)
        self.tokens = self.starts = None
        if entries[0][1] is not None:
            flat, starts, lens = ragged([t for _, t in entries])
            self.tokens, self.starts = torch.from_numpy(flat).to(device), torch.from_numpy(starts).to(device)
        else:
            lens = np.array([len(kv) for kv in kvs], np.int32)
        self.lengths, self.p_max = torch.from_numpy(lens).to(device), int(lens.max())
        self.ptrs = [[torch.tensor([kv.layers[l][j].data_ptr() for kv in kvs], dtype=torch.int64, device=device)
                      for j in range(2)] for l in range(len(p0.layers))]

    def cache_for(self, engine, pref_u):
        p0 = self.kvs[0]
        return DynamicCache(ddp_cache_data=[tuple(engine.gather_kv_padded(self.ptrs[l][j], self.lengths, pref_u, p0.heads,
                                                                           p0.head_dim, self.p_max, p0.dtype)
                                                  for j in range(2)) for l in range(len(p0.layers))])


class RaggedEncoding:

    def __init__(self, out, last):
        self.out, self.hidden, self.last = out, out.last_hidden_state, last

    def last_rows(self):
        return self.hidden[torch.arange(self.last.numel(), device=self.last.device), self.last.long()]

    def kv_layers(self):
        return [(ly.keys.contiguous(), ly.values.contiguous()) for ly in self.out.past_key_values.layers]


def encode_ragged(llm, batch, sel, n_sel, l_max, pad_id=0, base=None, prefixes=None, keep_kv=False):
    table, pref = prefixes or (None, None)
    eng = llm.engine
    ids, am, pos, last = eng.gather_padded(*batch, sel, n_sel, base, pad_id, 0 if table is None else table.p_max, l_max)
    cache = None if table is None else table.cache_for(eng, pref)
    return RaggedEncoding(llm._body(input_ids=ids, attention_mask=am, position_ids=pos, past_key_values=cache,
                                    use_cache=keep_kv or cache is not None), last)


PACKED_MAX_KEYS = 32


class PromptGroups:

    def __init__(self, prompts, device):
        if not prompts or any(len(p) < 1 for p in prompts):
            raise ValueError("a prompt group needs at least one token")
        self.lens = [len(p) for p in prompts]
        self.n_rows, self.p_max = sum(self.lens), max(self.lens)
        starts = np.concatenate([[0], np.cumsum(self.lens[:-1])]).astype(np.int32)
        lens = np.asarray(self.lens, np.int32)
        self.ids = torch.tensor([t for p in prompts for t in p], dtype=torch.int64, device=device)
        self.pos = torch.tensor([j for p in prompts for j in range(len(p))], dtype=torch.int64, device=device)
        self.starts_d, self.lens_d = torch.from_numpy(starts).to(device), torch.from_numpy(lens).to(device)
        zero = np.zeros_like(lens)
        self.segments = torch.from_numpy(np.stack([zero, zero, starts, lens], 1)).to(device)


def packed_plan(group_lens, grp, lens):
    group_lens, grp, lens = np.asarray(group_lens, np.int64), np.asarray(grp, np.int64), np.asarray(lens, np.int64)
    g_start = np.concatenate([[0], np.cumsum(group_lens[:-1])])
    n_pre = int(group_lens.sum())
    tail = lens - group_lens[grp]
    if (tail < 1).any():
        raise ValueError("every context needs a tail of at least one token behind its prompt")
    t_start = n_pre + np.concatenate([[0], np.cumsum(tail[:-1])])
    zero = np.zeros_like(group_lens)
    seg = np.concatenate([np.stack([zero, zero, g_start, group_lens], 1),
                          np.stack([g_start[grp], group_lens[grp], t_start, tail], 1)]).astype(np.int32)
    ctx = np.concatenate([np.repeat(-1 - np.arange(len(group_lens)), group_lens), np.repeat(np.arange(len(lens)), tail)])
    off = np.concatenate([np.arange(p) for p in group_lens] + [group_lens[grp[u]] + np.arange(tail[u]) for u in range(len(lens))])
    return seg, off.astype(np.int64), np.stack([ctx, off], 1).astype(np.int64), (t_start + tail - 1).astype(np.int64)


class _PackedLayer(CacheLayerMixin):

    is_compileable = False
    is_sliding = False

    def __init__(self, owner):
        super().__init__()
        self.owner = owner

    def lazy_initialization(self, key_states, value_states):
        self.is_initialized = True

    def update(self, key_states, value_states, *args, **kwargs):
        key_states._glb_packed = self.owner
        return key_states, value_states

    def get_mask_sizes(self, query_length):
        return query_length, 0

    def get_seq_length(self):
        return 0

    def get_max_length(self):
        return -1


class PackedKV(Cache):

    def __init__(self, engine, segments, n_rows, max_keys, n_layers):
        self.engine, self.segments, self.n_rows, self.max_keys = engine, segments, int(n_rows), int(max_keys)
        self.served = 0
        layer = _PackedLayer(self)
        super().__init__(layers=[layer] * n_layers)


class PackedEncoding:

    def __init__(self, out, last, n_rows):
        self.out, self.hidden, self.last, self.n_rows = out, out.last_hidden_state[0], last, n_rows

    def last_rows(self):
        return self.hidden[self.last]


def packed_supported(llm):
    body, eng = llm._body, llm.engine
    cfg = getattr(body, "config", None)
    if cfg is None or getattr(cfg, "_attn_implementation", None) != _ATTN_NAME or getattr(cfg, "_glb_engine", None) is not eng:
        return False
    heads = getattr(cfg, "num_attention_heads", None)
    head_dim = getattr(cfg, "head_dim", None) or (cfg.hidden_size // heads if heads else None)
    return bool(head_dim in (16, 32, 64, 128) and getattr(cfg, "num_hidden_layers", 0) > 0)


def encode_packed(llm, batch, sel, n_sel, grp, groups, n_tail_rows, max_keys=PACKED_MAX_KEYS):
    eng, dev = llm.engine, llm.device
    tokens, starts, lengths = batch
    if not 1 <= max_keys <= PACKED_MAX_KEYS:
        raise ValueError(f"encode_packed serves contexts of up to {PACKED_MAX_KEYS} tokens")
    if n_sel < 1 or n_tail_rows < n_sel:
        raise ValueError("encode_packed: every context feeds at least one tail row")
    if not packed_supported(llm):
        raise RuntimeError("encode_packed: this model's attention is not served by glb_short_attention")
    G, n_pre = len(groups.lens), groups.n_rows
    M = n_pre + int(n_tail_rows)
    sel_l, grp_l = sel[:n_sel].long(), grp[:n_sel].long().clamp(0, G - 1)
    pre_len, pre_start = groups.lens_d[grp_l], groups.starts_d[grp_l]
    tail = lengths[sel_l] - pre_len
    ends = torch.cumsum(tail, 0, dtype=torch.int32)
    tail_start = n_pre + ends - tail
    segments = torch.cat([groups.segments, torch.stack([pre_start, pre_len, tail_start, tail], 1)]).contiguous()
    r = torch.arange(int(n_tail_rows), dtype=torch.int32, device=dev)
    u = torch.searchsorted(ends, r, right=True).clamp_(max=n_sel - 1)
    pos_t = (pre_len[u] + (r - (ends - tail)[u])).long()
    at = (starts[sel_l[u]] + pos_t).clamp_(0, tokens.numel() - 1)
    ids = torch.cat([groups.ids, tokens[at].long()]).view(1, M)
    max_pos = getattr(llm._body.config, "max_position_embeddings", None) or (1 << 30)
    pos = torch.cat([groups.pos, pos_t.clamp_(0, min(PACKED_MAX_KEYS, max_pos) - 1)]).view(1, M)
    pkv = PackedKV(eng, segments, M, max_keys, llm._body.config.num_hidden_layers)
    out = llm._body(input_ids=ids, position_ids=pos, attention_mask=None, past_key_values=pkv, use_cache=True)
    if pkv.served != len(pkv.layers):
        raise RuntimeError(f"glb_short_attention_packed served {pkv.served} of {len(pkv.layers)} layers: an attention module "
                           "bypassed the attention interface and attended across the packed contexts")
    return PackedEncoding(out, (tail_start + tail - 1).long().clamp_(0, M - 1), M)


class PrefixLRU:

    def __init__(self, budget_bytes, on_remove=None):
        self.budget = int(budget_bytes)
        self.used = 0
        self._od = OrderedDict()
        self.evictions = 0
        self.on_remove = on_remove

    def put(self, node, kv):
        self.drop(node)
        size = kv.nbytes()
        node.past_key_values = kv
        self._od[id(node)] = (node, size)
        self.used += size
        while self.used > self.budget and len(self._od) > 1:
            _, (old, sz) = self._od.popitem(last=False)
            old.past_key_values = None
            self.used -= sz
            self.evictions += 1
            if self.on_remove is not None:
                self.on_remove(old)

    def touch(self, node):
        key = id(node)
        if key in self._od:
            self._od.move_to_end(key)

    def drop(self, node):
        ent = self._od.pop(id(node), None)
        if ent is not None:
            self.used -= ent[1]
            ent[0].past_key_values = None
            if self.on_remove is not None:
                self.on_remove(ent[0])

    def clear(self):
        nodes = [node for node, _ in self._od.values()]
        for node in nodes:
            node.past_key_values = None
        self._od.clear()
        self.used = 0
        if self.on_remove is not None:
            for node in nodes:
                self.on_remove(node)

    def nodes(self):
        return [node for node, _ in self._od.values()]

    def __len__(self):
        return len(self._od)
```

### genlm-backend_amd/sis.py

```python
import asyncio

import os

import numpy as np
import torch

from .cache import KVPrefix
from .fuse import SplitConv1D, split_gemm_all_rows
from .kv import PACKED_MAX_KEYS, PrefixTable, PromptGroups, SlabKV, SlabRunner, encode_packed, encode_ragged, packed_supported
from ._lib import MASK_BITS, MASK_NONE
from .masks import ParticleMasks

RNG_PHILOX, RNG_NOISE = 1, 2


def make_masks(llm, max_token_length):
    eos_id = llm.tokenizer.eos_token_id
    V = len(llm.byte_vocab)
    valid = torch.tensor([tid == eos_id or len(tok) <= max_token_length for tid, tok in enumerate(llm.byte_vocab)],
                         dtype=torch.float).log()
    eos_one_hot = torch.nn.functional.one_hot(torch.tensor(eos_id), V).log()
    masks = torch.stack([valid, eos_one_hot.to(torch.float)])
    llm.register_masks(masks)
    return masks


def make_masking_function(llm, max_token_length, max_tokens):
    make_masks(llm, max_token_length)
    return lambda context: 1 if len(context) >= max_tokens else 0


class Particle:

    def __init__(self, llm, mask_selector, prompt_ids, eos_id):
        self.context = []
        self.prompt_ids = prompt_ids
        self.log_weight = 0.0
        self.active = True
        self.llm = llm
        self.mask_selector = mask_selector
        self.eos_id = eos_id

    async def extend(self):
        logZ, token = await self.llm.next_token_step(self.prompt_ids + self.context,
                                                     mask_id=self.mask_selector(self.context))
        self.log_weight += logZ
        if token == self.eos_id or token < 0:
            self.active = False
        else:
            self.context.append(token)


async def autobatched_sis(n_particles, llm, mask_selector, prompt_ids, eos_id, gather=None):
    gather = gather or asyncio.gather
    particles = [Particle(llm, mask_selector, prompt_ids, eos_id) for _ in range(n_particles)]
    while any(p.active for p in particles):
        await gather(*[p.extend() for p in particles if p.active])
    return particles


def _gather_all(dist, out, inp):
    if inp.is_cuda and dist.get_backend() == "gloo":
        host = torch.empty(out.shape, dtype=out.dtype)
        dist.all_gather_into_tensor(host, inp.cpu())
        out.copy_(host)
    else:
        dist.all_gather_into_tensor(out, inp)


def _all_to_all(dist, out, inp, out_splits, in_splits):
    if inp.is_cuda and dist.get_backend() == "gloo":
        host = torch.empty(out.shape, dtype=out.dtype)
        dist.all_to_all_single(host, inp.cpu(), output_split_sizes=out_splits, input_split_sizes=in_splits)
        out.copy_(host)
    else:
        dist.all_to_all_single(out, inp, output_split_sizes=out_splits, input_split_sizes=in_splits)


def _all_to_all_any(dist, out, inp, out_splits, in_splits):
    if inp.is_cuda and dist.get_backend() == "gloo":
        host = torch.empty(out.shape, dtype=out.dtype)
        dist.all_to_all_single(host, inp.cpu(), output_split_sizes=out_splits, input_split_sizes=in_splits)
        out.copy_(host)
    else:
        dist.all_to_all_single(out, inp, output_split_sizes=out_splits, input_split_sizes=in_splits)


def _reduce_all(dist, t, op):
    if t.is_cuda and dist.get_backend() == "gloo":
        host = t.cpu()
        dist.all_reduce(host, op=op)
        t.copy_(host)
    else:
        dist.all_reduce(t, op=op)


class CollectiveClock:

    def __init__(self):
        self.on = False
        self.events, self.host_s, self.calls, self.bytes = [], 0.0, 0, 0

    def start(self):
        self.on = True
        self.events, self.host_s, self.calls, self.bytes = [], 0.0, 0, 0

    def run(self, fn, tensor, nbytes):
        if not self.on:
            return fn()
        self.calls += 1
        self.bytes += int(nbytes)
        if tensor.is_cuda and self._device_timed:
            e0, e1 = torch.cuda.Event(enable_timing=True), torch.cuda.Event(enable_timing=True)
            e0.record()
            out = fn()
            e1.record()
            self.events.append((e0, e1))
            return out
        import time

        t0 = time.perf_counter()
        out = fn()
        self.host_s += time.perf_counter() - t0
        return out

    _device_timed = True

    def total_us(self):
        return self.host_s * 1e6 + sum(a.elapsed_time(b) for a, b in self.events) * 1e3


class DeviceSIS:

    def __init__(self, llm, n_particles, prompt_ids, max_tokens, eos_id, seed=0, rng="philox", rank=0, world=1,
                 dist=None, use_prefix_kv=False, use_particle_kv=False, resample_ess=None, force_collectives=False,
                 share_kv=True, kv_rows=None, kv_in_place=0.75, kv_graph=True, particle_masks=None, migrate_kv=True,
                 constraint=None, share_prompt_rows=True, proposal_temperature=None, proposal=None):
        if constraint is not None and particle_masks is not None:
            raise ValueError("give particle_masks (the caller's bit rows) or constraint (masks made on the device), not both")
        self._propose = proposal_temperature is not None or proposal is not None
        if self._propose:
            if rng != "philox":
                raise ValueError(f"proposal_temperature / proposal need rng='philox', got rng={rng!r}: the reference has no draw "
                                 "from a proposal for the parity mode to be on par with")
            if proposal_temperature is not None and not float(proposal_temperature) > 0.0:
                raise ValueError(f"proposal_temperature must be > 0, got {proposal_temperature!r}")
            if proposal is not None:
                for flag, name in ((use_prefix_kv, "use_prefix_kv"), (use_particle_kv, "use_particle_kv")):
                    if flag:
                        raise ValueError(f"proposal= conflicts with {name}: a proposal model is served on the re-encoding path "
                                         "only (it keeps no KV rows)")
                vp, vq = int(llm.model.config.vocab_size), int(proposal.model.config.vocab_size)
                if vp != vq:
                    raise ValueError(f"proposal= has another vocabulary: {vq} tokens, the target {vp}")
                if proposal.device != llm.device:
                    raise ValueError(f"proposal= is on {proposal.device}, the target on {llm.device}")
        self.proposal = proposal
        self._q_scale = 1.0 if proposal_temperature is None else 1.0 / float(proposal_temperature)
        self._q_logits = None
        self.constraint = constraint
        self.llm, self.eng, self.dev = llm, llm.engine, llm.device
        self._lora_epoch = getattr(llm, "lora_epoch", 0)
        if hasattr(llm, "_lora_sync"):
            llm._lora_sync(self._lora_epoch)
        self.N, self.max_tokens, self.eos_id = n_particles, max_tokens, eos_id
        self.rank, self.world, self.dist = rank, world, dist
        self.collective = world > 1 or (bool(force_collectives) and dist is not None)
        self.coll_clock = CollectiveClock()
        if dist is not None:
            self.coll_clock._device_timed = dist.get_backend() != "gloo"
        self.rows_moved_total = 0
        self.migrate_kv = bool(migrate_kv)
        self.kv_rows_moved = 0
        self.seed = seed
        self.rng_mode = RNG_PHILOX if rng == "philox" else RNG_NOISE
        self.noise_src = None
        self.noise_ahead = os.environ.get("GLB_RNG_AHEAD", "0") == "1"
        prompts = prompt_ids if isinstance(prompt_ids[0], (list, tuple)) else [prompt_ids] * n_particles
        assert len(prompts) == n_particles
        self._prompt_len0 = torch.tensor([len(p) for p in prompts], dtype=torch.int32, device=self.dev)
        self.max_prompt = max(len(p) for p in prompts)
        if self.collective:
            mp_ = torch.tensor([self.max_prompt], dtype=torch.int64, device=self.dev)
            _reduce_all(dist, mp_, dist.ReduceOp.MAX)
            self.max_prompt = int(mp_.item())
        lens = {len(p) for p in prompts}
        if self.collective and resample_ess is not None:
            mm = torch.tensor([min(lens), -max(lens)], dtype=torch.int64, device=self.dev)
            _reduce_all(dist, mm, dist.ReduceOp.MIN)
            lens = {int(mm[0]), int(-mm[1])}
        self._mask_by_row = len(lens) == 1
        self._rep = None
        self.cap = self.max_prompt + max_tokens + 1
        ctx = np.zeros((n_particles, self.cap), np.int32)
        for i, p in enumerate(prompts):
            ctx[i, :len(p)] = p
        self._ctx0 = torch.from_numpy(ctx).to(self.dev)
        self.starts = (torch.arange(n_particles, device=self.dev, dtype=torch.int64) * self.cap)
        self.prefixes = None
        if use_prefix_kv:
            distinct = {tuple(p) for p in prompts}
            if self.collective and resample_ess is not None:
                width = self.max_prompt
                all_p = torch.empty((world * n_particles, width), dtype=torch.int32, device=self.dev)
                all_l = torch.empty(world * n_particles, dtype=torch.int32, device=self.dev)
                _gather_all(dist, all_p.view(-1), self._ctx0[:, :width].contiguous().view(-1))
                _gather_all(dist, all_l, self._prompt_len0)
                all_p, all_l = all_p.cpu().numpy(), all_l.cpu().numpy()
                distinct = {tuple(int(t) for t in all_p[i, :all_l[i]]) for i in range(len(all_l))}
            self._build_prefixes(sorted(distinct))
        self.particle_kv = bool(use_particle_kv)
        self.share_kv = bool(share_kv) and self.particle_kv
        self.share_prompt_rows = bool(share_prompt_rows)
        self.packed_steps = 0
        self._groups = self._grp0 = None
        if self.share_prompt_rows and not use_prefix_kv and not use_particle_kv and not (self.collective and world > 1):
            index = {}
            grp = [index.setdefault(tuple(p), len(index)) for p in prompts]
            self._groups = PromptGroups(list(index), self.dev)
            self._grp0 = torch.tensor(grp, dtype=torch.int32, device=self.dev)
        self.kv_rows = int(kv_rows) if kv_rows is not None else n_particles
        self.kv_stats = dict(forward_rows=0, encoded_rows=0, copied_rows=0, unkept_rows=0, steps=0, in_place_steps=0)
        self._kv = SlabRunner(llm, self.kv_rows, self.cap, kv_in_place, kv_graph)
        if self.particle_kv:
            assert not use_prefix_kv
        self._particle = ParticleMasks(self.eng, n_particles, particle_masks)
        self.constraint_raw_steps = 0
        self.rows_moved = 0
        self.resample_ess = resample_ess
        self.n_resamples = 0
        self.sync_every = 1
        self.reset()

    pkv = property(lambda self: self._kv.pkv)
    particle_masks = property(lambda self: self._particle.masks, lambda self, masks: setattr(self._particle, "masks", masks))
    pm_raw_above = property(lambda self: self._particle.raw_above, lambda self, frac: setattr(self._particle, "raw_above", frac))
    pm_raw_steps = property(lambda self: self._particle.raw_steps)
    _slab_fwd = property(lambda self: self._kv._slab_fwd)

    @torch.no_grad()
    def _build_prefixes(self, distinct):
        llm, dev = self.llm, self.dev
        entries = []
        for p in distinct:
            out = llm._body(input_ids=torch.tensor([list(p)], device=dev), use_cache=True)
            entries.append((KVPrefix.from_hf_cache(out.past_key_values), p))
        self.prefixes = PrefixTable(entries, dev)

    def reset(self):
        if self.noise_src is not None:
            self.noise_src.reset()
        self._particle.reset()
        self.contexts = self._ctx0.clone()
        self.prompt_len = self._prompt_len0.clone()
        self._grp = self._grp0
        self.lengths = self.prompt_len.clone()
        self.active = torch.ones(self.N, dtype=torch.int32, device=self.dev)
        self.log_weights = torch.full((self.N,), getattr(self.constraint, "start_logw", 0.0), dtype=torch.float32, device=self.dev)
        self.states =self.constraint.states0(self.N) if self.constraint is not None else None
        self.t = 0
        self.max_len_now = self.max_prompt
        self.last_stats = None
        self.kernel_events = []
        self.outer_events = []
        self._event_pool = []
        self._head_cache = None
        self._noise_buf = getattr(self, "_noise_buf", None)
        self._fwd_tokens = None
        self._noise_groups = None
        self._kv_stale = None
        self._row_of_d = torch.full((self.N,), -1, dtype=torch.int32, device=self.dev)
        self._global_active = torch.tensor(self.N * self.world, dtype=torch.int32, device=self.dev)
        self.all_weights = None
        self._all_stamp = None
        self._rehash()

    def _rehash(self):
        ctx_flat = self.contexts.view(-1)
        self.hashes = self.eng.hash_contexts(ctx_flat, self.starts, self.lengths)
        self._hash_stub = self.eng.hash_contexts(ctx_flat, self.starts, torch.ones_like(self.lengths))

    @torch.no_grad()
    def _encode_into_slabs(self, rows):
        eng, llm, dev, N = self.eng, self.llm, self.dev, self.N
        ctx_flat = self.contexts.view(-1)
        kv_len = self.lengths if self.t == 0 else (self.lengths - 1).clamp_min(1)
        want = torch.ones(N, dtype=torch.bool, device=dev) if rows is None else \
            torch.zeros(N, dtype=torch.bool, device=dev).index_fill_(0, rows, True)
        lens_eff = torch.where(want, kv_len, torch.ones_like(kv_len))
        group_of, rep, ng = eng.group_contexts(ctx_flat, self.starts, lens_eff)
        U = int(ng.item())
        l_max = int(lens_eff.max().item())
        enc = encode_ragged(llm, (ctx_flat, self.starts, lens_eff), rep, U, l_max, keep_kv=True)
        src = enc.kv_layers()
        if self.pkv is None:
            self._kv.pkv = SlabKV(eng, N, self.cap, len(src))
        src_row = torch.where(want, group_of, torch.full_like(group_of, -1))
        self.pkv.fill_rows(src, src_row, lens_eff)
        return enc, group_of, rep, U

    @torch.no_grad()
    def _step_particle_kv(self, time_kernel):
        eng, llm, dev, N = self.eng, self.llm, self.dev, self.N
        if self.t % self.sync_every == 0 or self._head_cache is None:
            head = torch.stack([self.active.sum().to(torch.int32), self._global_active, eng.error_word()[0]]).cpu()
            eng.raise_if_failed(int(head[2]))
            self._head_cache = (int(head[0]), int(head[1]))
        n_active, n_global = self._head_cache
        if self._kv_stale is not None:
            self._encode_into_slabs(torch.nonzero(self._kv_stale).flatten())
            self._kv_stale = None
        rows = torch.arange(N, device=dev)
        pos = (self.lengths - 1).clamp_min(0)
        newest = self.contexts[rows, pos.long()]
        ids = torch.where(self.active > 0, newest, torch.zeros_like(newest)).view(N, 1).long()
        logits = llm._lm_head(self._kv.slab_forward()(ids, pos))
        self._noise_groups = None
        if self.rng_mode == RNG_NOISE:
            lengths_eff = torch.where(self.active > 0, self.lengths, torch.ones_like(self.lengths))
            self._noise_groups, _, _ = eng.group_contexts(self.contexts.view(-1), self.starts, lengths_eff)
        return self._finish_step(logits, None, N, n_active, n_global, time_kernel, l_max=1)

    @torch.no_grad()
    def _step_shared_kv(self, time_kernel):
        eng, N, R = self.eng, self.N, self.kv_rows
        ctx_flat = self.contexts.view(-1)
        lengths_eff = torch.where(self.active > 0, self.lengths, torch.ones_like(self.lengths))
        hashes_eff = torch.where(self.active > 0, self.hashes, self._hash_stub)
        group_of, rep, ng = eng.group_contexts(ctx_flat, self.starts, lengths_eff, hashes=hashes_eff)
        plan = eng.kv_plan(group_of, rep, ng, self._row_of_d, lengths_eff, R, self.cap, by_context=True)
        head = torch.cat([plan["head"][:6], torch.stack([self.active.sum().to(torch.int32), self._global_active,
                                                          eng.error_word()[0]])]).cpu().tolist()
        U, nA, nB, n_copied, n_unkept, l_max_b, n_active, n_global = head[:8]
        eng.raise_if_failed(head[8])
        self._row_of_d = plan["row_of_context"]
        st = self.kv_stats
        st["forward_rows"] += U
        st["encoded_rows"] += nB
        st["copied_rows"] += n_copied
        st["unkept_rows"] += n_unkept
        st["steps"] += 1
        logits, self._fwd_tokens, in_place = self._kv.run(plan, head[:6], lambda ctx, pos: self.contexts[ctx, pos],
                                                          (ctx_flat, self.starts, lengths_eff))
        st["in_place_steps"] += int(in_place)
        self._rep = torch.cat([plan["ctx_a"][:nA], plan["ctx_b"][:nB]])
        self._noise_groups = group_of
        row_of = plan["logits_row"][group_of.long()]
        return self._finish_step(logits, row_of, U, n_active, n_global, time_kernel, l_max=1)

    def _finish_step(self, logits, group_of, U, n_active, n_global, time_kernel, l_max):
        eng, llm, N = self.eng, self.llm, self.N
        V = logits.shape[-1]
        mask_id = ((self.lengths - self.prompt_len) >= self.max_tokens).to(torch.int32)
        if self._propose:
            return self._finish_proposed(logits, group_of, U, n_active, n_global, time_kernel, l_max, mask_id)
        source = self.constraint if self.constraint is not None else self._particle if self.particle_masks is not None else llm.masks
        kw, raw = source.step_masks(logits, *self._mask_units(logits, group_of, mask_id), N, parity=self.rng_mode == RNG_NOISE)
        self.constraint_raw_steps += int(raw and self.constraint is not None)
        if self.rng_mode == RNG_NOISE:
            kw["noise"] = self._parity_noise(self._noise_groups if self._noise_groups is not None else group_of, V)
        if time_kernel:
            if len(self._event_pool) < 2:
                self._event_pool = eng.timing_events(64)
            inner, (e0, e1) = self._event_pool.pop(), self._event_pool.pop()
            e0.record()
            kw["timing_events"] = inner
        logZ, _, tok = eng.step(logits, vocab=V, row_of=group_of, rng_mode=self.rng_mode, seed=self.seed,
                                offset=self.t, particle_base=self.rank * N, want_lse=False, **kw)
        if time_kernel:
            e1.record()
            self.kernel_events.append(inner)
            self.outer_events.append((e0, e1))
        if self.rng_mode == RNG_NOISE:
            self.noise_src.prefetch()
        return self._advance(logits, mask_id, logZ, tok, U, n_active, n_global, l_max)

    def _proposal_masks(self, logits, ids, by_row):
        key = "row_mask_id" if by_row else "mask_id"
        if self.constraint is not None:
            kw, raw = self.constraint.step_masks(logits, ids, by_row, self.N, parity=False)
            self.constraint_raw_steps += int(raw)
            return kw
        if self.particle_masks is not None:
            return {"mask_kind": MASK_BITS, "mask": self.particle_masks, key: ids}
        m = self.llm.masks
        return {} if m.kind == MASK_NONE else {"mask_kind": m.kind, "mask": m.table, key: ids}

    def _finish_proposed(self, logits, group_of, U, n_active, n_global, time_kernel, l_max, mask_id):
        eng, N = self.eng, self.N
        kw = self._proposal_masks(logits, *self._mask_units(logits, group_of, mask_id))
        q, self._q_logits = self._q_logits, None
        if time_kernel:
            if len(self._event_pool) < 2:
                self._event_pool = eng.timing_events(64)
            e0, e1 = self._event_pool.pop()
            e0.record()
        dlogw, tok, _ = eng.importance_step(logits, q, proposal_scale=self._q_scale, vocab=logits.shape[-1], row_of=group_of,
                                            seed=self.seed, offset=self.t, particle_base=self.rank * N, **kw)
        if time_kernel:
            e1.record()
            self.kernel_events.append((e0, e1))
            self.outer_events.append((e0, e1))
        return self._advance(logits, mask_id, dlogw, tok, U, n_active, n_global, l_max)

    def _advance(self, logits, mask_id, logZ, tok, U, n_active, n_global, l_max):
        eng = self.eng
        len_was = self.lengths.clone() if self.constraint is not None else None
        if self.constraint is not None and self.constraint.weighted:
            self.log_weights += self.constraint.forced_final_logw(self.states, (mask_id > 0) & (self.active > 0) & (tok == self.eos_id))
        eng.particles_advance(self.contexts, self.lengths, self.active, self.log_weights, logZ, tok, self.eos_id,
                              self.cap, hashes=self.hashes)
        if self.constraint is not None:
            self.constraint.advance(self.states, self.contexts, len_was, self.lengths, out=self.states)
        self.t += 1
        self.max_len_now = min(self.max_len_now + 1, self.cap)
        ft = self._fwd_tokens if self._fwd_tokens is not None else U * l_max
        self._fwd_tokens = None
        self.last_stats = dict(n_unique=U, n_active=n_active, l_max=l_max, n_rows=U, fwd_tokens=ft, head_rows=logits.shape[0])
        self._exchange()
        if self.resample_ess is not None:
            self._maybe_resample()
        return U, n_global

    def _mask_units(self, logits, group_of, done):
        if self.constraint is None and self.particle_masks is not None:
            own = torch.arange(self.N, dtype=torch.int32, device=self.dev)
            return torch.where(done > 0, torch.full_like(own, self.N), own), False
        ids = done if self.constraint is None else self.constraint.mask_rows(self.states, done=done)
        if self._mask_by_row and group_of is not None:
            ids = ids[self._rep[:logits.shape[0]].long()].contiguous()
        return ids, self._mask_by_row

    def _recompute_states(self):
        if self.constraint is not None:
            self.states = self.constraint.advance(None, self.contexts, self.prompt_len, self.lengths)

    def update_particle_masks(self, rows, bit_rows):
        self._particle.update(rows, bit_rows)

    def _exchange(self):
        count = self.active.sum().to(torch.float32).view(1)
        if self.collective:
            N = self.N
            parts = [self.log_weights, count]
            carry = self.rng_mode == RNG_NOISE and self.world > 1
            if carry:
                parts += [self.hashes.view(torch.float32), self.active.to(torch.float32)]
            mine = torch.cat(parts)
            out = torch.empty((self.world, mine.numel()), dtype=torch.float32, device=self.dev)
            self.coll_clock.run(lambda: _gather_all(self.dist, out.view(-1), mine), mine, out.numel() * 4)
            self.all_weights = out[:, :N].reshape(-1)
            self._global_active = out[:, N].sum().to(torch.int32)
            if carry:
                self._all_hashes = out[:, N + 1:3 * N + 1].contiguous().view(torch.int64).reshape(-1)
                self._all_active = out[:, 3 * N + 1:].reshape(-1) > 0
                self._all_stamp = (self.t, self.n_resamples)
        else:
            self.all_weights = self.log_weights
            self._global_active = count[0].to(torch.int32)

    @torch.no_grad()
    def step(self, time_kernel=False):
        eng, llm, dev, N = self.eng, self.llm, self.dev, self.N
        if hasattr(llm, "_lora_sync"):
            llm._lora_sync(self._lora_epoch)
        if self.share_kv:
            return self._step_shared_kv(time_kernel)
        if self.particle_kv and self.t > 0:
            return self._step_particle_kv(time_kernel)
        ctx_flat = self.contexts.view(-1)
        lengths_eff = torch.where(self.active > 0, self.lengths, torch.ones_like(self.lengths))
        if self.particle_kv:
            head = torch.stack([self.active.sum().to(torch.int32), self._global_active, eng.error_word()[0]]).cpu()
            n_active, n_global = int(head[0]), int(head[1])
            eng.raise_if_failed(int(head[2]))
            enc, group_of, rep, U = self._encode_into_slabs(None)
            self._rep = rep
            self._noise_groups = None
            return self._finish_step(llm._lm_head(enc.last_rows()), group_of, U, n_active, n_global, time_kernel, self.max_len_now)
        hashes_eff = torch.where(self.active > 0, self.hashes, self._hash_stub)
        group_of, rep, ng = eng.group_contexts(ctx_flat, self.starts, lengths_eff, hashes=hashes_eff)
        self._rep = rep
        head = torch.stack([ng[0], self.active.sum().to(torch.int32), self._global_active, eng.error_word()[0]]).cpu()
        U, n_active, n_global = int(head[0]), int(head[1]), int(head[2])
        eng.raise_if_failed(int(head[3]))
        base, prefixes = None, None
        l_max = self.max_len_now
        if self.prefixes is not None and self.t > 0:
            P = self.prefixes
            pref, base = eng.match_prefixes(ctx_flat, self.starts, lengths_eff, P.tokens, P.starts, P.lengths)
            prefixes = (P, pref[rep[:U].long()].contiguous())
            l_max = max(self.t, 1)
        if self._packed_ready(U, n_active, l_max):
            with split_gemm_all_rows(eng):
                enc = encode_packed(llm, (ctx_flat, self.starts, lengths_eff), rep, U, self._grp[rep[:U].long()],
                                    self._groups, U * self.t, max_keys=l_max)
            self._fwd_tokens = enc.n_rows
            self.packed_steps += 1
        else:
            enc = encode_ragged(llm, (ctx_flat, self.starts, lengths_eff), rep, U, l_max, base=base, prefixes=prefixes)
        logits = llm._lm_head(enc.last_rows())
        if self.proposal is not None:
            other = self.proposal
            self._q_logits = other._lm_head(encode_ragged(other, (ctx_flat, self.starts, lengths_eff), rep, U, l_max).last_rows())
        self._noise_groups = None
        return self._finish_step(logits, group_of, U, n_active, n_global, time_kernel, l_max)

    def _packed_ready(self, U, n_active, l_max):
        if self._groups is None or self.t < 1 or n_active != self.N or l_max > PACKED_MAX_KEYS or self.prefixes is not None:
            return False
        body = self.llm._body
        ent = self.__dict__.get("_packed_body")
        if ent is None or ent[0] is not body:
            rows = [m.min_rows for m in body.modules() if isinstance(m, SplitConv1D)]
            ent = self._packed_body = (body, max(rows) if rows and packed_supported(self.llm) else None)
        return ent[1] is not None and U * l_max >= ent[1]

    def _parity_noise(self, group_of, V):
        N = self.N
        if self.noise_src is None:
            self.noise_src = self.eng.noise_rng(self.seed, V, ahead=self.noise_ahead and self.world == 1)
        if self.collective and self.world > 1:
            return self._parity_noise_sharded(V)
        act = self.active > 0
        key = torch.where(act, group_of.to(torch.int64), torch.full((N,), 1 << 40, dtype=torch.int64, device=self.dev))
        order = torch.argsort(key, stable=True)
        rank = torch.empty(N, dtype=torch.int32, device=self.dev)
        rank[order] = torch.arange(N, dtype=torch.int32, device=self.dev)
        slot = torch.where(act, rank, torch.full_like(rank, -1))
        if self._noise_buf is None or self._noise_buf.shape != (N, V):
            self._noise_buf = torch.empty((N, V), dtype=torch.float32, device=self.dev)
        return self.noise_src.rows(N, row_slot=slot, n_draw=act.sum().to(torch.int32), max_draw=N, out=self._noise_buf)

    def _parity_noise_sharded(self, V):
        N, dev = self.N, self.dev
        if getattr(self, "_all_stamp", None) != (self.t, self.n_resamples):
            mine = torch.cat([self.hashes.view(torch.float32), self.active.to(torch.float32)])
            out = torch.empty((self.world, 3 * N), dtype=torch.float32, device=dev)
            self.coll_clock.run(lambda: _gather_all(self.dist, out.view(-1), mine), mine, out.numel() * 4)
            self._all_hashes = out[:, :2 * N].contiguous().view(torch.int64).reshape(-1)
            self._all_active = out[:, 2 * N:].reshape(-1) > 0
            self._all_stamp = (self.t, self.n_resamples)
        h, act = self._all_hashes, self._all_active
        NT = h.numel()
        ar = torch.arange(NT, device=dev)
        sh, perm = torch.sort(h, stable=True)
        start = torch.ones(NT, dtype=torch.bool, device=dev)
        start[1:] = sh[1:] != sh[:-1]
        first = perm[torch.cummax(torch.where(start, ar, torch.zeros_like(ar)), 0).values]
        key = torch.empty(NT, dtype=torch.int64, device=dev)
        key[perm] = first
        key = torch.where(act, key, torch.full_like(key, 1 << 40))
        order = torch.argsort(key, stable=True)
        place = torch.empty(NT, dtype=torch.int32, device=dev)
        place[order] = torch.arange(NT, dtype=torch.int32, device=dev)
        slot = torch.where(act, place, torch.full_like(place, -1))[self.rank * N:(self.rank + 1) * N].contiguous()
        if self._noise_buf is None or self._noise_buf.shape != (N, V):
            self._noise_buf = torch.empty((N, V), dtype=torch.float32, device=dev)
        return self.noise_src.rows(N, row_slot=slot, n_draw=act.sum().to(torch.int32), max_draw=NT, out=self._noise_buf)

    def gather_weights(self):
        if self.all_weights is None:
            self._exchange()
        return self.all_weights

    def normalized_weights(self):
        return self.eng.normalize_weights(self.gather_weights())

    @torch.no_grad()
    def _maybe_resample(self):
        n_total = self.N * self.world
        if self.resample_ess < 1.0:
            _, stats = self.eng.normalize_weights(self.all_weights)
            if float(stats[1].item()) >= self.resample_ess * n_total:
                return
        self.resample()

    @torch.no_grad()
    def resample(self):
        eng, N, dev = self.eng, self.N, self.dev
        n_total = N * self.world
        anc, lse = eng.resample_systematic(self.all_weights, self.seed ^ 0x5eed5a11, self.t)
        mine = anc[self.rank * N:(self.rank + 1) * N].contiguous()
        state = torch.cat([self.contexts, torch.stack([self.lengths, self.prompt_len, self.active], dim=1)], dim=1).contiguous()
        local = mine - self.rank * N
        new_state = eng.gather_rows_i32(state, local.clamp(0, N - 1))
        if self.collective and self.world > 1:
            anc_h = anc.cpu().numpy()
            owner = anc_h // N
            r = self.rank
            send_idx = [anc_h[d * N:(d + 1) * N][owner[d * N:(d + 1) * N] == r] - r * N if d != r else anc_h[:0]
                        for d in range(self.world)]
            mine_owner = owner[r * N:(r + 1) * N]
            recv_cnt = [int((mine_owner == src).sum()) if src != r else 0 for src in range(self.world)]
            self.rows_moved = int((owner != np.repeat(np.arange(self.world), N)).sum())
            self.rows_moved_total += self.rows_moved
            moved = None
            if self.rows_moved:
                take = np.concatenate(send_idx).astype(np.int64)
                take_d = torch.from_numpy(take).to(dev)
                send = state[take_d] if len(take) else state[:0]
                recv = torch.empty((sum(recv_cnt), state.shape[1]), dtype=torch.int32, device=dev)
                send_cnt = [len(x) for x in send_idx]
                send = send.contiguous()
                self.coll_clock.run(lambda: _all_to_all(self.dist, recv, send, recv_cnt, send_cnt), send,
                                    (send.numel() + recv.numel()) * 4)
                slots_d = None
                if sum(recv_cnt):
                    slots = np.concatenate([np.nonzero(mine_owner == src)[0] for src in range(self.world) if src != r])
                    slots_d = torch.from_numpy(slots.astype(np.int64)).to(dev)
                    new_state[slots_d] = recv
                moved = (take_d, send_cnt, slots_d, recv_cnt)
        self.contexts = new_state[:, :self.cap].contiguous()
        self.lengths, self.prompt_len, self.active = (new_state[:, self.cap + k].contiguous() for k in range(3))
        self.log_weights = (lse - float(np.log(n_total))).expand(N).contiguous()
        if self._grp is not None:
            self._grp = self._grp[local.clamp(0, N - 1).long()]
        if self.share_kv:
            local = mine - self.rank * N
            ok = (local >= 0) & (local < N)
            self._row_of_d = torch.where(ok, self._row_of_d[local.clamp(0, N - 1).long()], torch.full_like(local, -1))
        elif self.particle_kv and self.pkv is not None:
            local = mine - self.rank * N
            is_local = (local >= 0) & (local < N)
            src = torch.where(is_local, local, torch.full_like(local, -1))
            kv_len = (self.lengths - 1).clamp_min(0)
            self.pkv.gather(src, kv_len)
            stale = ~is_local
            if self.migrate_kv and self.collective and self.world > 1:
                if self.rows_moved:
                    self._migrate_kv(*moved)
                self._kv_stale = None
            else:
                self._kv_stale = stale if bool(stale.any().item()) else None
        self._rehash()
        self._recompute_states()
        self.n_resamples += 1
        self._exchange()

    def _migrate_kv(self, take_d, send_cnt, slots_d, recv_cnt):
        pkv = self.pkv
        new = pkv._tensors(pkv.layers)
        old = pkv._alt
        n_send, n_recv = int(sum(send_cnt)), int(sum(recv_cnt))
        shape = tuple(new[0].shape[1:])
        for t in new:
            if tuple(t.shape[1:]) != shape or t.dtype != new[0].dtype:
                raise ValueError("KV layers of different shapes: rows cannot travel in one message")
        send = torch.stack([t[take_d] for t in old], dim=1).contiguous() if n_send else new[0].new_zeros((0, len(new)) + shape)
        recv = new[0].new_empty((n_recv, len(new)) + shape)
        self.coll_clock.run(lambda: _all_to_all_any(self.dist, recv, send, recv_cnt, send_cnt), send,
                            (send.numel() + recv.numel()) * send.element_size())
        if n_recv:
            for j, t in enumerate(new):
                t[slots_d] = recv[:, j]
        self.kv_rows_moved += n_recv

    @torch.no_grad()
    def run(self, max_steps=None):
        steps = 0
        limit = max_steps if max_steps is not None else self.max_tokens + 1
        while steps < limit:
            _, n_global = self.step()
            steps += 1
            if n_global == 0:
                break
        return steps

    @torch.no_grad()
    def rescore(self, llm=None, prompt_ids=None, constraint=None):
        llm = self.llm if llm is None else llm
        gen = self.lengths - self.prompt_len
        drew_eos = (self.active == 0) & torch.isfinite(self.log_weights) & (self.lengths < self.cap)
        at_end = self.lengths.clamp(max=self.cap - 1).long()[:, None]
        last = torch.where(drew_eos[:, None], torch.full_like(at_end, self.eos_id), self.contexts.gather(1, at_end))
        tokens = self.contexts.scatter(1, at_end, last.to(torch.int32))
        lengths, plen = self.lengths + drew_eos.to(torch.int32), self.prompt_len
        forced_at = None
        if constraint is not None:
            forced_at = torch.where(drew_eos & (gen >= self.max_tokens), gen, torch.full_like(gen, -1))
        if prompt_ids is not None:
            prompt = torch.tensor(list(prompt_ids), dtype=torch.int32, device=self.dev)
            if prompt.numel() == 0:
                raise ValueError("a prompt needs at least one token")
            n_p = prompt.numel()
            j = torch.arange(n_p + self.cap, device=self.dev)[None] - n_p
            own = torch.gather(tokens, 1, (plen[:, None].long() + j).clamp(0, self.cap - 1))
            shared = prompt[(j + n_p).clamp(min=0, max=n_p - 1)].expand(self.N, -1)
            tokens = torch.where(j < 0, shared, own).contiguous()
            plen = torch.full_like(plen, n_p)
            lengths = plen + gen + drew_eos.to(torch.int32)
        return llm.batch_sequence_logprobs_device(tokens, lengths, plen, constraint=constraint, forced_at=forced_at)

    def results(self):
        self.eng.check()
        if self.constraint is not None:
            self.constraint.check()
        ctx = self.contexts.cpu().numpy()
        ln = self.lengths.cpu().numpy()
        pl = self.prompt_len.cpu().numpy()
        return [list(ctx[i, pl[i]:ln[i]]) for i in range(self.N)], self.log_weights.cpu().numpy()


class DeviceSampler(DeviceSIS):

    def __init__(self, llm, prompts, max_tokens, eos_token_ids, temperature=1.0, seed=None, sync_every=4):
        super().__init__(llm, len(prompts), [list(p) for p in prompts], max_tokens, eos_id=-1,
                         seed=0 if seed is None else int(seed), rng="philox", use_particle_kv=True, share_kv=False,
                         kv_graph=max_tokens >= 64)
        self.sync_every = max(1, int(sync_every))
        self.temperature = float(temperature)
        self.eos = torch.tensor(sorted(set(int(t) for t in eos_token_ids)), dtype=torch.int32, device=self.dev)
        self.seeded = seed is not None
        if not self.seeded:
            self.seed = int(torch.randint(0, 2**62, (1,)).item())

    def _finish_step(self, logits, group_of, U, n_active, n_global, time_kernel, l_max):
        eng, N, dev = self.eng, self.N, self.dev
        V = logits.shape[-1]
        kw = {}
        mode = RNG_PHILOX
        if self.seeded:
            mode = RNG_NOISE
            if self.noise_src is None:
                self.noise_src = eng.noise_rng(self.seed, V)
            kw["noise"] = self.noise_src.rows(1)
        _, _, tok = eng.step(logits, vocab=V, row_of=group_of, rng_mode=mode, seed=self.seed, offset=self.t,
                             logit_scale=1.0 / self.temperature, want_lse=False, **kw)
        act = (self.active > 0) & (tok != -2)
        stop = act & (torch.isin(tok, self.eos) | (tok < 0) | (self.lengths - self.prompt_len >= self.max_tokens))
        keep = act & ~stop
        rows = torch.arange(N, device=dev)
        at = self.lengths.long().clamp_max(self.cap - 1)
        self.contexts[rows, at] = torch.where(keep, tok, self.contexts[rows, at])
        self.lengths = self.lengths + keep.to(torch.int32)
        self.active = torch.where(tok == -2, self.active, (keep & (self.lengths - self.prompt_len < self.max_tokens)).to(torch.int32))
        self.t += 1
        self.max_len_now = min(self.max_len_now + 1, self.cap)
        self._exchange()
        return U, n_global

    def generate(self):
        steps = 0
        while steps < self.max_tokens:
            _, n_global = self.step()
            steps += 1
            if n_global == 0:
                break
        return self.results()[0]


class SisBenchWorkload:

    def __init__(self, eng, dev, rank, world, dist, n_particles=1024, max_tokens=10, prefix_kv=False, particle_kv=False,
                 model="gpt2", n_prompts=1, resample=False, force_collectives=False, kv_in_place=0.75,
                 per_particle_masks=False, rng="philox", gemms="library", share_prompt_rows=True):
        from .llm import AsyncAmdLM

        if model == "gpt2":
            from transformers import GPT2Config

            cfg, dtype = GPT2Config(), torch.float32
            self.model_name = "gpt2-small shape (random init, fp32)"
        elif model == "llama-3-8b":
            from transformers import LlamaConfig

            cfg = LlamaConfig(vocab_size=128256, hidden_size=4096, intermediate_size=14336, num_hidden_layers=32,
                              num_attention_heads=32, num_key_value_heads=8, head_dim=128, max_position_embeddings=4096,
                              rope_theta=500000.0, rms_norm_eps=1e-5, tie_word_embeddings=False, bos_token_id=128000,
                              eos_token_id=128001)
            dtype = torch.bfloat16
            self.model_name = "Llama-3-8B shape (random init, bf16)"
        else:
            from transformers import LlamaConfig

            cfg = LlamaConfig(vocab_size=128256, hidden_size=2048, intermediate_size=8192, num_hidden_layers=16,
                              num_attention_heads=32, num_key_value_heads=8, head_dim=64, max_position_embeddings=4096,
                              rope_theta=500000.0, rms_norm_eps=1e-5, tie_word_embeddings=True, bos_token_id=128000,
                              eos_token_id=128001)
            dtype = torch.bfloat16
            self.model_name = "Llama-3.2-1B shape (random init, bf16)"
        self.dtype_name = "f32" if dtype == torch.float32 else "bf16"
        self.elem = 4 if dtype == torch.float32 else 2
        self.llm = AsyncAmdLM.from_config(cfg, None, device=dev, dtype=dtype, seed=1234, engine=eng,
                                          batch_size=n_particles, gemms=gemms)
        V = cfg.vocab_size
        g = torch.Generator(device=dev)
        g.manual_seed(4321)
        valid = torch.where(torch.rand(V, device=dev, generator=g) < 1 / 3, float("-inf"), 0.0)
        valid[cfg.eos_token_id] = 0.0
        eos1 = torch.full((V,), float("-inf"), device=dev)
        eos1[cfg.eos_token_id] = 0.0
        self.llm.register_masks(torch.stack([valid, eos1]))
        pm = None
        if per_particle_masks:
            own = torch.where(torch.rand((n_particles, V), device=dev, generator=g) < 1 / 3, float("-inf"), 0.0)
            own[:, cfg.eos_token_id] = 0.0
            pm, _ = eng.mask_to_bits(torch.cat([own, eos1[None]]))
            del own
        self.per_particle_masks = per_particle_masks
        self.V, self.N, self.max_tokens = V, n_particles, max_tokens
        self.particles_per_step = n_particles
        rs = np.random.default_rng(99)
        base = [list(range(100, 108))] + [[int(t) for t in rs.integers(1000, 30000, 8)] for _ in range(n_prompts - 1)]
        prompts = [base[i % n_prompts] for i in range(n_particles)] if n_prompts > 1 else base[0]
        self.n_prompts = n_prompts
        self.rng = rng
        self.sis = DeviceSIS(self.llm, n_particles, prompts, max_tokens, cfg.eos_token_id,
                             seed=1234, rng=rng, rank=rank, world=world, dist=dist, use_prefix_kv=prefix_kv,
                             use_particle_kv=particle_kv, resample_ess=1.0 if resample else None,
                             force_collectives=force_collectives, kv_in_place=kv_in_place, particle_masks=pm,
                             share_prompt_rows=share_prompt_rows)
        self.prefix_kv = prefix_kv
        self.particle_kv = particle_kv
        self.resample = resample
        self.kernel_bytes = None
        self._events = []
        self._outer = []
        self._bytes = []
        self.unique_hist = []
        self.fed_hist = []
        self.flops_hist = []
        body = self.llm._body
        self._lin_w = sum(m.weight.numel() for m in body.modules() if type(m).__name__ in ("Linear", "Conv1D", "SplitConv1D"))
        self._lin_w += sum(m.in_features * m.out_features for m in body.modules() if type(m).__name__ == "W4Linear")
        self._head_w = self.llm._head.weight.numel()
        for _ in range(max_tokens):
            self.sis.step(time_kernel=False)
        self.sis.reset()
        torch.cuda.synchronize(dev)

    def step(self, i, timed):
        if self.sis.t >= self.max_tokens:
            self._collect()
            self.sis.reset()
        U, _ = self.sis.step(time_kernel=timed)
        if timed:
            n_masks = self.N + 1 if self.per_particle_masks else 2
            self._bytes.append(U * self.V * self.elem + n_masks * ((self.V + 31) // 32) * 4 + self.N * 8
                               + (self.N * self.V * 4 if self.rng != "philox" else 0))
            self.unique_hist.append(U)
            self.fed_hist.append(int(self.sis.last_stats["l_max"]))
            ls = self.sis.last_stats
            self.flops_hist.append(2.0 * self._lin_w * ls["fwd_tokens"] + 2.0 * self._head_w * ls["head_rows"])

    def _collect(self):
        self._events.extend(self.sis.kernel_events)
        self._outer.extend(self.sis.outer_events)
        self.sis.kernel_events = []
        self.sis.outer_events = []

    def kernel_times_us(self):
        self._collect()
        self.kernel_bytes = float(np.mean(self._bytes)) if self._bytes else 0.0
        self.kernel_bytes_each = np.array(self._bytes, dtype=np.float64)
        return np.array([a.elapsed_time(b) * 1e3 for a, b in self._events])

    def keep_kernel_times(self, n):
        self._collect()
        for name in ("_events", "_outer", "_bytes", "unique_hist", "fed_hist", "flops_hist"):
            setattr(self, name, getattr(self, name)[:n])

    def outer_times_us(self):
        return np.array([a.elapsed_time(b) * 1e3 for a, b in self._outer])

    def config(self):
        return {"workload": f"SIS step: {self.N} particles/GPU, {self.model_name}, prompt len 8, <=10 new "
                            "tokens, " + (f"{self.N} per-particle bit masks (standing still: handed over raw at the first step, prepared from the second on)" if self.per_particle_masks
                                          else "2 shared bit masks") + ", device-resident population, "
                            + ("Philox draws" if self.rng == "philox" else "the reference's draws (torch.multinomial's CPU MT19937 stream, "
                               "generated on the device: ids identical to torch's under the seed)")
                            + (f", {self.n_prompts} distinct shared prompts" if self.n_prompts > 1 else "")
                            + (", prompt KV cached (cache_kv semantics, BASELINE config 3)" if self.prefix_kv else "")
                            + (", device-resident KV rows shared by particles with equal contexts (one new token per distinct "
                               "context per step; NOT the reference's re-encode-every-step algorithm)" if self.particle_kv else "")
                            + (", systematic resampling after every step" if self.resample else ""),
                "particles_per_gpu": self.N, "vocab": self.V,
                "rng": "philox" if self.rng == "philox" else "parity (torch CPU generator on the device)",
                "mean_unique_contexts_per_step": float(np.mean(self.unique_hist)) if self.unique_hist else None,
                "mean_tokens_fed_per_context": float(np.mean(self.fed_hist)) if self.fed_hist else None,
                "gemm_flops_per_step": float(np.mean(self.flops_hist)) if self.flops_hist else None,
                **({"prefixed_tokens_per_context": 8} if self.prefix_kv else {}),
                **({"kv_rows": {k: v for k, v in self.sis.kv_stats.items()}} if self.particle_kv else {})}
```

### include/glb.h

```cpp
#ifndef GLB_H
#define GLB_H

#include <stddef.h>
#include <stdint.h>

#ifdef __cplusplus
extern "C" {
#endif

#define GLB_ABI_VERSION 9

enum {
  GLB_OK = 0,
  GLB_EINVAL = 1,
  GLB_EUNSUPPORTED = 2,
  GLB_EHIP = 3,
  GLB_ENOSPC = 4
};

enum { GLB_F32 = 0, GLB_BF16 = 1, GLB_F16 = 2 };

enum {
  GLB_MASK_NONE = 0,
  GLB_MASK_BITS = 1,
  GLB_MASK_F32 = 2,
  GLB_MASK_PREPARED = 3
};

enum { GLB_STEP_HW_EXP = 1 };

enum {
  GLB_RNG_NONE = 0,
  GLB_RNG_PHILOX = 1,
  GLB_RNG_NOISE = 2
};

const char *glb_version(void);
int glb_abi_version(void);
int glb_last_error(char *buf, size_t n);
int glb_device_count(void);

typedef struct glb_step_args {
  uint32_t struct_size;
  const void *logits;
  int32_t dtype;
  int64_t n_rows;
  int64_t vocab;
  int64_t ld;
  float logit_scale;
  int64_t n_particles;
  const int32_t *row_of;
  int32_t mask_kind;
  const void *mask;
  int64_t mask_ld;
  int64_t n_masks;
  const int32_t *mask_id;
  const int32_t *row_mask_id;
  int32_t rng_mode;
  const float *noise;
  int64_t noise_ld;
  uint64_t seed;
  uint64_t offset;
  int64_t particle_base;
  float *out_logZ;
  float *out_lse;
  int32_t *out_token;
  float *out_margin;
  int32_t flags;
  void *workspace;
  size_t workspace_bytes;
} glb_step_args;

size_t glb_step_workspace_bytes(int64_t n_particles, int64_t n_rows, int64_t vocab, int64_t n_masks);
int glb_logprob_mask_sample(const glb_step_args *args, void *hip_stream);
int glb_logprob_mask_sample_timed(const glb_step_args *args, void *hip_stream, void *start_event, void *stop_event);

int glb_workspace_init(void *workspace, size_t workspace_bytes, void *hip_stream);
int glb_workspace_release(void *workspace);
int glb_workspace_check(void *workspace, void *hip_stream);
const uint32_t *glb_workspace_error_word(void *workspace);
#define GLB_SPIN_NONE UINT64_MAX
int glb_set_spin_limit(uint64_t microseconds);

size_t glb_mask_prepared_bytes(int64_t n_masks, int64_t vocab);
int glb_mask_prepare(const uint32_t *mask_bits, int64_t n_masks, int64_t vocab, int64_t mask_ld, int32_t dtype,
                     void *out_prepared, size_t out_bytes, void *hip_stream);
int glb_mask_prepare_rows(const uint32_t *mask_bits, int64_t n_masks, int64_t vocab, int64_t mask_ld, int32_t dtype,
                          const int32_t *rows, int64_t n_rows, void *prepared, size_t prepared_bytes, void *hip_stream);

size_t glb_log_softmax_workspace_bytes(int64_t n_rows, int64_t vocab);
int glb_log_softmax_rows(const void *logits, int32_t dtype, int64_t n_rows, int64_t vocab,
                         int64_t ld, float logit_scale, void *out_logprobs, int32_t out_dtype, int64_t out_ld,
                         float *out_lse, void *workspace, size_t workspace_bytes, void *hip_stream);

int glb_mask_f32_to_bits(const float *mask, int64_t n_masks, int64_t vocab, int64_t mask_ld,
                         uint32_t *out_bits, int64_t bits_ld, int32_t *out_nonbinary,
                         void *hip_stream);

size_t glb_group_contexts_workspace(int64_t n);
int glb_group_contexts(const int32_t *tokens, const int64_t *starts, const int32_t *lengths,
                       int64_t n, const uint64_t *ctx_hashes, int32_t *out_group_of, int32_t *out_rep,
                       int32_t *out_n_groups, void *workspace, size_t workspace_bytes, void *hip_stream);
int glb_hash_contexts(const int32_t *tokens, const int64_t *starts, const int32_t *lengths, int64_t n,
                      uint64_t *out_hashes, void *hip_stream);

int glb_match_prefixes(const int32_t *tokens, const int64_t *starts, const int32_t *lengths,
                       int64_t n, const int32_t *prefix_tokens, const int64_t *prefix_starts,
                       const int32_t *prefix_lengths, int64_t n_prefixes, int32_t *out_prefix,
                       int32_t *out_base, void *hip_stream);

int glb_gather_padded(const int32_t *tokens, const int64_t *starts, const int32_t *lengths,
                      const int32_t *sel, int64_t n_sel, const int32_t *base, int64_t pad_id, int64_t p_max,
                      int64_t l_max, int64_t *out_input_ids, int64_t *out_attention_mask,
                      int64_t *out_position_ids, int32_t *out_last_index, void *hip_stream);

int glb_gather_kv_padded(const void *const *slabs, const int32_t *slab_len, int64_t n_prefixes,
                         const int32_t *prefix_of, int64_t n_rows, int64_t heads,
                         int64_t head_dim, int64_t p_max, int32_t elem_bytes, void *out,
                         void *hip_stream);

int glb_particles_advance(int32_t *contexts, int64_t ctx_ld, int32_t *lengths, int32_t *active,
                          float *log_weights, const float *logZ, const int32_t *token, int64_t n,
                          int32_t eos_id, int32_t max_len, uint64_t *ctx_hashes, void *hip_stream);

int glb_normalize_weights(const float *log_weights, int64_t n, float *out_probs, float *out_stats,
                          void *hip_stream);

int glb_kv_append(void *slab, const void *new_rows, const int32_t *pos, const int32_t *row_of, int64_t n_rows,
                  int64_t heads, int64_t cap, int64_t head_dim, int64_t new_stride_row, int64_t new_stride_head,
                  int32_t elem_bytes, void *hip_stream);
int glb_kv_gather_rows(const void *const *src, void *const *dst, int64_t n_tensors, int64_t n_rows, int64_t heads,
                       int64_t head_dim, int64_t src_cap, int64_t dst_cap, const int32_t *src_row_of,
                       const int32_t *len_of, int32_t elem_bytes, void *hip_stream);
int glb_gather_rows_i32(const int32_t *src, int64_t src_ld, const int32_t *row_of, int64_t n, int64_t width,
                        int32_t *dst, int64_t dst_ld, void *hip_stream);

int glb_match_rows(const int32_t *tokens, const int64_t *starts, const int32_t *lengths, const int32_t *rep,
                   const int32_t *n_groups, int64_t n, const int32_t *row_tok, const int32_t *row_len,
                   const uint64_t *row_hash, int64_t n_rows, int64_t cap, int32_t *out_old_row, uint64_t *out_hash,
                   void *hip_stream);
typedef struct glb_kv_plan_args {
  uint32_t struct_size;
  int64_t n, n_rows, cap;
  const int32_t *group_of, *rep, *n_groups;
  const int32_t *old_row;
  int32_t old_row_by_context;
  const int32_t *lengths;
  int64_t *row_stamps;
  int64_t call_no;
  int32_t *row_tok, *row_len;
  uint64_t *row_hash;
  const uint64_t *group_hash;
  const int32_t *tokens;
  const int64_t *starts;
  int32_t *out_group_row, *out_logits_row, *out_rows_a, *out_ctx_a, *out_pos_a, *out_ctx_b, *out_rows_b, *out_copy_src,
      *out_copy_len, *out_ctx_of_row, *out_pos_of_row, *out_row_of_context, *out_head;
  void *workspace;
  size_t workspace_bytes;
} glb_kv_plan_args;
size_t glb_kv_plan_workspace(int64_t n, int64_t n_rows);
int glb_kv_plan(const glb_kv_plan_args *args, void *hip_stream);

#define GLB_KV_CHUNK_MAX 16
int glb_match_prefix_rows(const int32_t *tokens, const int64_t *starts, const int32_t *lengths, const int32_t *rep,
                          const int32_t *n_groups, int64_t n, const int32_t *row_tok, const int32_t *row_len,
                          const uint64_t *row_hash, int64_t n_rows, int64_t cap, int32_t max_new, int32_t *out_old_row,
                          int32_t *out_keep, uint64_t *out_hash, void *hip_stream);
typedef struct glb_kv_plan_chunk_args {
  uint32_t struct_size;
  glb_kv_plan_args plan;
  const int32_t *old_keep;
  int32_t *out_n_new_a, *out_n_new_of_row;
} glb_kv_plan_chunk_args;
int glb_kv_plan_chunk(const glb_kv_plan_chunk_args *args, void *hip_stream);
int glb_slab_attention_chunk(const void *q, const int64_t q_strides[3], const void *k_new, const int64_t k_strides[3],
                             const void *v_new, const int64_t v_strides[3], void *k_slab, void *v_slab, const int32_t *pos,
                             const int32_t *n_new, const int32_t *row_of, int64_t n_rows, int64_t n_slab_rows, int64_t heads,
                             int64_t kv_heads, int64_t cap, int64_t head_dim, int64_t max_new, float scale, int32_t dtype,
                             void *out, void *hip_stream);

int glb_slab_attention(const void *q, int64_t q_stride_row, int64_t q_stride_head, const void *k_new, int64_t k_stride_row,
                       int64_t k_stride_head, const void *v_new, int64_t v_stride_row, int64_t v_stride_head, void *k_slab,
                       void *v_slab, const int32_t *pos,
                       int64_t n_rows, int64_t heads, int64_t kv_heads, int64_t cap, int64_t head_dim, float scale,
                       int32_t dtype, void *out, void *hip_stream);

int glb_short_attention(const void *q, const int64_t q_strides[3], const void *k, const int64_t k_strides[3], const void *v,
                        const int64_t v_strides[3], const uint8_t *mask, int64_t mask_stride_row, int64_t mask_stride_query,
                        int64_t n_rows, int64_t heads, int64_t kv_heads, int64_t q_len, int64_t k_len, int64_t head_dim,
                        float scale, int32_t dtype, void *out, void *hip_stream);

int glb_short_attention_packed(const void *q, int64_t q_stride_row, int64_t q_stride_head, const void *k, int64_t k_stride_row,
                               int64_t k_stride_head, const void *v, int64_t v_stride_row, int64_t v_stride_head,
                               const int32_t *plan, int64_t n_segments, int64_t n_rows, int64_t heads, int64_t kv_heads,
                               int64_t max_keys, int64_t head_dim, float scale, int32_t dtype, void *out, uint32_t *err_word,
                               void *hip_stream);

size_t glb_resample_workspace(int64_t n);
int glb_resample_systematic(const float *log_weights, int64_t n, uint64_t seed, uint64_t offset,
                            int32_t *out_ancestors, float *out_stats, void *workspace, size_t workspace_bytes,
                            void *hip_stream);

enum { GLB_TRIE_SUM = 0, GLB_TRIE_MAX = 1 };
size_t glb_trie_workspace(int64_t n_rows, int64_t n_nodes);
int glb_trie_reduce(const float *weights, int64_t ld, int64_t n_rows, int64_t vocab, int64_t n_nodes, int64_t n_levels,
                    const int32_t *leaf_node, const int32_t *level_start_host, const int32_t *level_nodes,
                    const int32_t *child_ptr, const int32_t *child_idx, int32_t op, int32_t from_logprobs, float *out,
                    int64_t out_ld, void *workspace, size_t workspace_bytes, void *hip_stream);

typedef struct glb_trie_args {
  uint32_t struct_size;
  const void *weights;
  int32_t dtype;
  int64_t ld, n_rows, vocab;
  const float *lse;
  float logit_scale;
  int32_t from_logprobs;
  int32_t op;
  int64_t n_nodes, n_levels;
  const int32_t *leaf_node, *level_start_host, *level_nodes, *child_ptr, *child_idx;
  float *out;
  int64_t out_ld;
  const int32_t *sel_nodes;
  int64_t n_sel;
  float *out_sel;
  int64_t out_sel_ld;
  int32_t keep_node_major;
  void *workspace;
  size_t workspace_bytes;
} glb_trie_args;
size_t glb_trie_workspace_ex(int64_t n_rows, int64_t n_nodes);
int glb_trie_masses(const glb_trie_args *args, void *hip_stream);

typedef struct glb_trie_plan {
  uint32_t struct_size;
  int32_t n_parts, n_top, n_cut, n_slots, max_local, top_base, lds_bytes;
  int64_t n_nodes;
  const int32_t *desc, *idepth, *leaf_src, *leaf_local, *run_tab, *top_local, *slot_of;
  const uint16_t *cptr16, *inode16, *pn_local16;
  const uint16_t *tok_local16;
  const uint64_t *inode64;
  int32_t lds_top_bytes, vocab;
} glb_trie_plan;
typedef struct glb_trie_rows_args {
  uint32_t struct_size;
  const void *weights;
  int32_t dtype;
  int64_t ld, n_rows, vocab;
  const float *lse;
  float logit_scale;
  int32_t from_logprobs;
  int32_t op;
  float *out_slots;
  int64_t out_slots_ld;
  float *out_nodes;
  int64_t out_nodes_ld;
  const int32_t *sel_nodes;
  int64_t n_sel;
  float *out_sel;
  int64_t out_sel_ld;
  void *workspace;
  size_t workspace_bytes;
  int64_t sel_row_stride;
} glb_trie_rows_args;
size_t glb_trie_rows_workspace(int64_t n_rows, const glb_trie_plan *plan);
int glb_trie_rows(const glb_trie_rows_args *args, const glb_trie_plan *plan, void *hip_stream);

typedef struct glb_mt19937 {
  uint32_t mt[624];
  int32_t idx;
} glb_mt19937;
void glb_mt19937_seed(glb_mt19937 *st, uint64_t seed);
int glb_mt19937_exponential_f32(glb_mt19937 *st, float *out, int64_t n);

#define GLB_MT_POLY_WORDS 312
int glb_mt19937_window(uint64_t seed, uint32_t *out_window );
// ... 309 lines not shown
int glb_nfa_closure(const glb_nfa_args *args, void *hip_stream);
int glb_nfa_subset_round(const glb_nfa_args *args, void *hip_stream);

#define GLB_LAZY_STATUS 8
#define GLB_LAZY_OVERFLOW 1
#define GLB_LAZY_BUG 2
typedef struct glb_lazy_args {
  uint32_t struct_size;
  glb_dfa_args dfa;
  int32_t n_nfa_states, nfa_start;
  int32_t n_important, n_words;
  int32_t n_arcs;
  int32_t max_states;
  const int32_t *arc_off, *arc_dst;
  const uint64_t *arc_bytes;
  const uint64_t *accepting_mask;
  const uint64_t *eclose;
  uint64_t hash_mask;
  void *table;
  int64_t table_slots;
  uint64_t *cand;
  int32_t *counts;
  int64_t cand_rows;
  uint64_t *sets;
  uint8_t *accepting_out;
  int32_t *status;
  int32_t *row_state, *row_stamp, *claimants, *victims;
  int32_t *ecounters;
  int32_t *epoch;
  int32_t force_wave;
} glb_lazy_args;
int glb_lazy_init(const glb_lazy_args *args, void *hip_stream);
int glb_lazy_advance(const glb_lazy_args *args, void *hip_stream);
int glb_lazy_serve(const glb_lazy_args *args, void *hip_stream);

#define GLB_PDA_MAX_DEPTH 504
#define GLB_PDA_STATUS 8
#define GLB_PDA_OVERFLOW 1
#define GLB_PDA_BUG 2
typedef struct glb_pda_args {
  uint32_t struct_size;
  glb_dfa_args dfa;
  int32_t n_pda_states, n_symbols, start;
  int32_t max_depth, n_words, max_states;
  const int32_t *delta;
  const uint8_t *accepting;
  uint64_t hash_mask;
  void *table;
  int64_t table_slots;
  uint64_t *cand;
  int32_t *counts;
  int64_t cand_rows;
  uint64_t *configs;
  uint8_t *accepting_out;
  int32_t *status;
  int32_t *row_state, *row_stamp, *claimants, *victims;
  int32_t *ecounters;
  int32_t *epoch;
  int32_t max_token_bytes;
} glb_pda_args;
int glb_pda_init(const glb_pda_args *args, void *hip_stream);
int glb_pda_advance(const glb_pda_args *args, void *hip_stream);
int glb_pda_serve(const glb_pda_args *args, void *hip_stream);

#define GLB_CONJ_MAX_PARTS 8
#define GLB_CONJ_STATUS 8
#define GLB_CONJ_OVERFLOW 1
#define GLB_CONJ_BUG 2
typedef struct glb_conj_args {
  uint32_t struct_size;
  glb_dfa_args dfa;
  int32_t n_parts, n_words, max_states;
  int32_t part_start[GLB_CONJ_MAX_PARTS];
  uint64_t hash_mask;
  void *table;
  int64_t table_slots;
  uint64_t *tuples;
  int32_t *status;
  int32_t *counts;
  int64_t cand_rows;
  int32_t *part_states;
  int64_t part_ld;
  int32_t *claim_states;
  int32_t *rep;
  const int32_t *part_rows[GLB_CONJ_MAX_PARTS];
  const void *part_bank[GLB_CONJ_MAX_PARTS];
  int64_t part_bank_ld[GLB_CONJ_MAX_PARTS], part_capacity[GLB_CONJ_MAX_PARTS];
  int32_t part_weighted[GLB_CONJ_MAX_PARTS];
  float *wbank;
  int64_t wbank_ld;
  int32_t *row_state, *row_stamp, *claimants, *victims;
  int32_t *ecounters;
  int32_t *epoch;
} glb_conj_args;
int glb_conj_init(const glb_conj_args *args, void *hip_stream);
int glb_conj_unpack(const glb_conj_args *args, void *hip_stream);
int glb_conj_number(const glb_conj_args *args, void *hip_stream);
int glb_conj_serve(const glb_conj_args *args, void *hip_stream);

typedef struct glb_importance_args {
  uint32_t struct_size;
  const void *target;
  int32_t target_dtype;
  int64_t ld_p;
  const void *proposal;
  int32_t proposal_dtype;
  int64_t ld_q;
  int64_t n_rows, vocab;
  float proposal_scale;
  int64_t n_particles;
  const int32_t *row_of;
  int32_t mask_kind;
  const void *mask;
  int64_t mask_ld, n_masks;
  const int32_t *mask_id;
  const int32_t *row_mask_id;
  uint64_t seed, offset;
  int64_t particle_base;
  int32_t *out_token;
  float *out_dlogw;
  float *out_lse_target;
  float *out_logZ_proposal;
  void *workspace;
  size_t workspace_bytes;
} glb_importance_args;
size_t glb_importance_workspace_bytes(int64_t n_particles, int64_t n_rows, int64_t vocab);
int glb_importance_step(const glb_importance_args *args, void *hip_stream);

typedef struct glb_score_args {
  uint32_t struct_size;
  const void *logits;
  int32_t dtype;
  int64_t n_rows, vocab;
  int64_t ld;
  float logit_scale;
  const int32_t *token;
  int32_t mask_kind;
  const void *mask;
  int64_t mask_ld, n_masks;
  const int32_t *row_mask_id;
  float *out_logp;
  float *out_lse;
  float *out_logZ;
  float *out_logp_masked;
  const int64_t *seq_start;
  int64_t n_seq;
  float *out_seq_logp;
  float *out_seq_logZ;
  float *out_seq_logp_masked;
} glb_score_args;
int glb_score_rows(const glb_score_args *args, void *hip_stream);
int glb_score_seq_sums(const float *values, int64_t n_rows, const int64_t *seq_start, int64_t n_seq, float *out, void *hip_stream);

void glb_philox4x32_10(const uint32_t ctr[4], const uint32_t key[2], uint32_t out[4]);

#ifdef __cplusplus
}
#endif
#endif
```

Baseline: 142,600.

## Fuse particle advance with step-state derivation and add device packed-plan kernels

```diff
diff --git a/genlm-backend_amd/_lib.py b/genlm-backend_amd/_lib.py
--- a/genlm-backend_amd/_lib.py
+++ b/genlm-backend_amd/_lib.py
@@ -486,6 +486,24 @@
         ("out_seq_logp", C.c_void_p), ("out_seq_logZ", C.c_void_p), ("out_seq_logp_masked", C.c_void_p),
     ]
 
+
+class PackedPlanArgs(C.Structure):
+    _fields_ = [
+        ("struct_size", C.c_uint32),
+        ("tokens", C.c_void_p), ("starts", C.c_void_p), ("lengths", C.c_void_p),
+        ("n_tokens", C.c_int64), ("n_ctx", C.c_int64),
+        ("sel", C.c_void_p), ("grp", C.c_void_p), ("n_sel", C.c_int64),
+        ("group_lens", C.c_void_p), ("group_starts", C.c_void_p), ("group_segments", C.c_void_p),
+        ("group_ids", C.c_void_p), ("group_pos", C.c_void_p),
+        ("n_groups", C.c_int64), ("n_pre", C.c_int64),
+        ("n_tail_rows", C.c_int64),
+        ("max_keys", C.c_int32),
+        ("pos_bound", C.c_int64),
+        ("out_segments", C.c_void_p), ("out_ids", C.c_void_p), ("out_pos", C.c_void_p), ("out_last_rows", C.c_void_p),
+    ]
+
+
+PACKED_PLAN_MAX_SEL = 1 << 20
 
 _vp, _i32, _i64, _f32, _sz = C.c_void_p, C.c_int32, C.c_int64, C.c_float, C.c_size_t
 SYMBOLS = {
@@ -603,6 +621,9 @@
     "glb_importance_step": (C.c_int, [C.POINTER(ImportanceArgs), _vp]),
     "glb_score_rows": (C.c_int, [C.POINTER(ScoreArgs), _vp]),
     "glb_score_seq_sums": (C.c_int, [_vp, _i64, _vp, _i64, _vp, _vp]),
+    "glb_particles_advance2": (C.c_int, [_vp, _i64, _vp, _vp, _vp, _vp, _vp, _i64, _i32, _i32, _vp, _vp, _vp, _i32,
+                                         _vp, _vp, _vp, _vp, _i32, _vp]),
+    "glb_packed_plan": (C.c_int, [C.POINTER(PackedPlanArgs), _vp]),
     "glb_philox4x32_10": (None, [C.POINTER(C.c_uint32), C.POINTER(C.c_uint32), C.POINTER(C.c_uint32)]),
 }
 
diff --git a/genlm-backend_amd/csrc/glb_api.hip b/genlm-backend_amd/csrc/glb_api.hip
--- a/genlm-backend_amd/csrc/glb_api.hip
+++ b/genlm-backend_amd/csrc/glb_api.hip
@@ -547,6 +547,57 @@
     len[i] = l + 1;
     if (hashes) hashes[i] = ctx_hash_step(hashes[i], (uint32_t)t);
     if (l + 1 >= max_len) active[i] = 0;
+  }
+}
+
+struct Advance2Out {
+  const int32_t *prompt_len;
+  const uint64_t *hash_stub;
+  int32_t max_tokens, to_global;
+  int32_t *lengths_eff;
+  uint64_t *hashes_eff;
+  int32_t *done, *head;
+};
+
+__global__ __launch_bounds__(256) void particles_advance2_kernel(int32_t *ctx, int64_t ctx_ld, int32_t *len, int32_t *active,
+                                                                 float *lw, const float *logZ, const int32_t *tok, int64_t n,
+                                                                 int32_t eos, int32_t max_len, uint64_t *hashes,
+                                                                 const Advance2Out o) {
+  __shared__ int32_t block_sum;
+  if (threadIdx.x == 0) block_sum = 0;
+  __syncthreads();
+  const int64_t i = (int64_t)blockIdx.x * 256 + threadIdx.x;
+  if (i < n) {
+    int32_t act = active[i], l = len[i];
+    uint64_t h = hashes[i];
+    const int32_t t = tok[i];
+    if (act && t != -2) {
+      lw[i] += logZ[i];
+      if (t == eos || t < 0) {
+        active[i] = act = 0;
+      } else {
+        ctx[i * ctx_ld + l] = t;
+        len[i] = l = l + 1;
+        hashes[i] = h = ctx_hash_step(h, (uint32_t)t);
+        if (l >= max_len) active[i] = act = 0;
+      }
+    }
+    o.lengths_eff[i] = act > 0 ? l : 1;
+    o.hashes_eff[i] = act > 0 ? h : o.hash_stub[i];
+    o.done[i] = (int32_t)((uint32_t)l - (uint32_t)o.prompt_len[i]) >= o.max_tokens ? 1 : 0;
+    if (act) atomicAdd(&block_sum, act);
+  }
+  __syncthreads();
+  if (threadIdx.x == 0) {
+    atomicAdd(&o.head[4], block_sum);
+    __threadfence();
+    if (atomicAdd(&o.head[5], 1) == (int32_t)gridDim.x - 1) {
+      __threadfence();
+      const int32_t total = atomicExch(&o.head[4], 0);
+      o.head[1] = total;
+      if (o.to_global) o.head[2] = total;
+      atomicExch(&o.head[5], 0);
+    }
   }
 }
 
@@ -1064,6 +1115,25 @@
   return GLB_OK;
 }
 
+int glb_particles_advance2(int32_t *contexts, int64_t ctx_ld, int32_t *lengths, int32_t *active, float *log_weights,
+                           const float *logZ, const int32_t *token, int64_t n, int32_t eos_id, int32_t max_len,
+                           uint64_t *hashes, const int32_t *prompt_len, const uint64_t *hash_stub, int32_t max_tokens,
+                           int32_t *out_lengths_eff, uint64_t *out_hashes_eff, int32_t *out_done, int32_t *head,
+                           int32_t to_global, void *stream) {
+  if (!contexts || !lengths || !active || !log_weights || !logZ || !token || !hashes || !prompt_len || !hash_stub)
+    return fail(GLB_EINVAL, "null pointer");
+  if (!out_lengths_eff || !out_hashes_eff || !out_done || !head) return fail(GLB_EINVAL, "null output pointer");
+  if (n <= 0 || n > 0x7fffffffll || ctx_ld <= 0 || max_len > ctx_ld) return fail(GLB_EINVAL, "bad sizes");
+  Advance2Out o;
+  o.prompt_len = prompt_len, o.hash_stub = hash_stub, o.max_tokens = max_tokens, o.to_global = to_global;
+  o.lengths_eff = out_lengths_eff, o.hashes_eff = out_hashes_eff, o.done = out_done, o.head = head;
+  hipLaunchKernelGGL(particles_advance2_kernel, dim3(blocks_for(n, 256)), dim3(256), 0, (hipStream_t)stream, contexts, ctx_ld,
+                     lengths, active, log_weights, logZ, token, n, eos_id, max_len, hashes, o);
+  const hipError_t e = hipGetLastError();
+  if (e != hipSuccess) return hip_fail(e, "particles_advance2 launch");
+  return GLB_OK;
+}
+
 void glb_philox4x32_10(const uint32_t ctr[4], const uint32_t key[2], uint32_t out[4]) {
   glb::philox4x32_10(ctr, key, out);
 }
diff --git a/genlm-backend_amd/csrc/glb_plan.hip b/genlm-backend_amd/csrc/glb_plan.hip
--- /dev/null
+++ b/genlm-backend_amd/csrc/glb_plan.hip
@@ -0,0 +1,142 @@
+#include <hip/hip_runtime.h>
+
+#include <cstdint>
+
+#include "../../include/glb.h"
+#include "glb_common.hpp"
+
+namespace {
+using namespace glb;
+
+constexpr int kScanThreads = 1024;
+constexpr int kScanWaves = kScanThreads / 64;
+
+struct PlanParams {
+  const int32_t *tokens;
+  const int64_t *starts;
+  const int32_t *lengths;
+  const int32_t *sel, *grp;
+  const int32_t *group_lens, *group_starts, *group_segments;
+  const int64_t *group_ids, *group_pos;
+  int64_t n_tokens, n_ctx, n_sel, n_groups, n_pre, n_rows, pos_bound;
+  int32_t *segments;
+  int64_t *ids, *pos, *last_rows;
+};
+
+__device__ __forceinline__ int64_t context_of(const PlanParams &p, int64_t u) {
+  int64_t s = p.sel[u];
+  if (s < 0) s += p.n_ctx;
+  return s < 0 ? 0 : (s >= p.n_ctx ? p.n_ctx - 1 : s);
+}
+
+__device__ __forceinline__ int64_t group_of(const PlanParams &p, int64_t u) {
+  const int64_t g = p.grp[u];
+  return g < 0 ? 0 : (g >= p.n_groups ? p.n_groups - 1 : g);
+}
+
+__global__ __launch_bounds__(kScanThreads) void plan_scan_kernel(const PlanParams p) {
+  __shared__ uint32_t wave_sum[kScanWaves];
+  const int tid = threadIdx.x, lane = tid & 63, wave = tid >> 6;
+  for (int64_t i = tid; i < p.n_groups * 4; i += kScanThreads) p.segments[i] = p.group_segments[i];
+  const uint32_t n_pre = (uint32_t)p.n_pre;
+  uint32_t carry = 0;
+  for (int64_t base = 0; base < p.n_sel; base += kScanThreads) {
+    const int64_t u = base + tid;
+    uint32_t tail = 0, pre_len = 0, pre_start = 0;
+    if (u < p.n_sel) {
+      const int64_t g = group_of(p, u);
+      pre_len = (uint32_t)p.group_lens[g];
+      pre_start = (uint32_t)p.group_starts[g];
+      tail = (uint32_t)p.lengths[context_of(p, u)] - pre_len;
+    }
+    uint32_t incl = tail;
+    for (int d = 1; d < 64; d <<= 1) {
+      const uint32_t o = __shfl_up(incl, d, 64);
+      if (lane >= d) incl += o;
+    }
+    if (lane == 63) wave_sum[wave] = incl;
+    __syncthreads();
+    uint32_t before = carry, total = carry;
+    for (int w = 0; w < kScanWaves; ++w) {
+      const uint32_t s = wave_sum[w];
+      if (w < wave) before += s;
+      total += s;
+    }
+    __syncthreads();
+    carry = total;
+    if (u < p.n_sel) {
+      const uint32_t ends = before + incl, tail_start = n_pre + ends - tail;
+      int32_t *seg = p.segments + (p.n_groups + u) * 4;
+      seg[0] = (int32_t)pre_start;
+      seg[1] = (int32_t)pre_len;
+      seg[2] = (int32_t)tail_start;
+      seg[3] = (int32_t)tail;
+      const int64_t last = (int32_t)(tail_start + tail - 1u);
+      p.last_rows[u] = last < 0 ? 0 : (last >= p.n_rows ? p.n_rows - 1 : last);
+    }
+  }
+}
+
+__global__ __launch_bounds__(256) void plan_rows_kernel(const PlanParams p) {
+  const int64_t m = (int64_t)blockIdx.x * 256 + threadIdx.x;
+  if (m >= p.n_rows) return;
+  if (m < p.n_pre) {
+    p.ids[m] = p.group_ids[m];
+    p.pos[m] = p.group_pos[m];
+    return;
+  }
+  const int32_t *seg = p.segments + p.n_groups * 4;
+  const uint32_t n_pre = (uint32_t)p.n_pre;
+  const int32_t r = (int32_t)(m - p.n_pre);
+  int64_t lo = 0, hi = p.n_sel;
+  while (lo < hi) {
+    const int64_t mid = lo + ((hi - lo) >> 1);
+    const int32_t ends = (int32_t)((uint32_t)seg[mid * 4 + 2] + (uint32_t)seg[mid * 4 + 3] - n_pre);
+    if (!(ends > r)) lo = mid + 1;
+    else hi = mid;
+  }
+  const int64_t u = lo > p.n_sel - 1 ? p.n_sel - 1 : lo;
+  const uint32_t tail_start = (uint32_t)seg[u * 4 + 2];
+  const int64_t pos_t = (int32_t)((uint32_t)seg[u * 4 + 1] + ((uint32_t)r - (tail_start - n_pre)));
+  int64_t at = p.starts[context_of(p, u)] + pos_t;
+  at = at < 0 ? 0 : (at >= p.n_tokens ? p.n_tokens - 1 : at);
+  p.ids[m] = (int64_t)p.tokens[at];
+  p.pos[m] = pos_t < 0 ? 0 : (pos_t >= p.pos_bound ? p.pos_bound - 1 : pos_t);
+}
+
+}
+
+extern "C" {
+
+int glb_packed_plan(const glb_packed_plan_args *a, void *stream) {
+  const char *const what = "glb_packed_plan";
+  if (int rc = block_ok(a, what, "glb_packed_plan_args")) return rc;
+  if (!a->tokens || !a->starts || !a->lengths || !a->sel || !a->grp) return api_fail(GLB_EINVAL, "%s: null batch pointer", what);
+  if (!a->group_lens || !a->group_starts || !a->group_segments || !a->group_ids || !a->group_pos)
+    return api_fail(GLB_EINVAL, "%s: null prompt-group pointer", what);
+  if (!a->out_segments || !a->out_ids || !a->out_pos || !a->out_last_rows) return api_fail(GLB_EINVAL, "%s: null output pointer", what);
+  if (a->n_tokens < 1 || a->n_ctx < 1 || a->n_sel < 1 || a->n_groups < 1 || a->n_pre < 1 || a->n_tail_rows < 0)
+    return api_fail(GLB_EINVAL, "%s: n_tokens=%lld n_ctx=%lld n_sel=%lld n_groups=%lld n_pre=%lld n_tail_rows=%lld", what,
+                    (long long)a->n_tokens, (long long)a->n_ctx, (long long)a->n_sel, (long long)a->n_groups, (long long)a->n_pre,
+                    (long long)a->n_tail_rows);
+  if (a->max_keys < 1 || a->max_keys > 32) return api_fail(GLB_EINVAL, "%s: max_keys %d outside [1, 32]", what, a->max_keys);
+  if (a->pos_bound < 1) return api_fail(GLB_EINVAL, "%s: pos_bound %lld must be positive", what, (long long)a->pos_bound);
+  if (a->n_sel > GLB_PACKED_PLAN_MAX_SEL)
+    return api_fail(GLB_EUNSUPPORTED, "%s: n_sel %lld above %d (one workgroup scans the tails)", what, (long long)a->n_sel,
+                    GLB_PACKED_PLAN_MAX_SEL);
+  if (a->n_groups > 0x7fffffffll / 8 || a->n_pre > 0x3fffffffll || a->n_tail_rows > 0x3fffffffll)
+    return api_fail(GLB_EINVAL, "%s: rows exceed 31 bits", what);
+  PlanParams p;
+  p.tokens = a->tokens, p.starts = a->starts, p.lengths = a->lengths, p.sel = a->sel, p.grp = a->grp;
+  p.group_lens = a->group_lens, p.group_starts = a->group_starts, p.group_segments = a->group_segments;
+  p.group_ids = a->group_ids, p.group_pos = a->group_pos;
+  p.n_tokens = a->n_tokens, p.n_ctx = a->n_ctx, p.n_sel = a->n_sel, p.n_groups = a->n_groups, p.n_pre = a->n_pre;
+  p.n_rows = a->n_pre + a->n_tail_rows, p.pos_bound = a->pos_bound;
+  p.segments = a->out_segments, p.ids = a->out_ids, p.pos = a->out_pos, p.last_rows = a->out_last_rows;
+  hipStream_t s = (hipStream_t)stream;
+  hipLaunchKernelGGL(plan_scan_kernel, dim3(1), dim3(kScanThreads), 0, s, p);
+  hipLaunchKernelGGL(plan_rows_kernel, dim3(blocks_for(p.n_rows, 256)), dim3(256), 0, s, p);
+  return launched("glb_packed_plan launch");
+}
+
+}
diff --git a/genlm-backend_amd/engine.py b/genlm-backend_amd/engine.py
--- a/genlm-backend_amd/engine.py
+++ b/genlm-backend_amd/engine.py
@@ -13,6 +13,20 @@
 
 def _ptr(t):
     return None if t is None else C.c_void_p(t.data_ptr())
+
+
+def check_advance2_args(contexts, lengths, active, log_weights, logZ, token, hashes, prompt_len, hash_stub, head):
+    if contexts.dim() != 2 or contexts.dtype != torch.int32:
+        raise ValueError("particles_advance2: contexts must be int32 [n, ld]")
+    n, ld = contexts.shape
+    for name, t, dt in (("lengths", lengths, torch.int32), ("active", active, torch.int32), ("log_weights", log_weights, torch.float32),
+                        ("logZ", logZ, torch.float32), ("token", token, torch.int32), ("hashes", hashes, torch.int64),
+                        ("prompt_len", prompt_len, torch.int32), ("hash_stub", hash_stub, torch.int64)):
+        if t is None or t.dtype != dt or t.numel() != n:
+            raise ValueError(f"particles_advance2: {name} must be {dt} [{n}]")
+    if head is None or head.dtype != torch.int32 or head.numel() < 6:
+        raise ValueError("particles_advance2: head must hold at least six int32 words")
+    return n, ld
 
 
 class LoraRowsTable:
@@ -603,13 +617,15 @@
         check(self.lib.glb_hash_contexts(_ptr(tokens), _ptr(starts), _ptr(lengths), n, _ptr(out), self._stream()))
         return out
 
-    def group_contexts(self, tokens, starts, lengths, hashes=None):
+    def group_contexts(self, tokens, starts, lengths, hashes=None, out=None):
         n = lengths.numel()
-        self._check_dev(tokens, starts, lengths, hashes)
+        self._check_dev(tokens, starts, lengths, hashes, out)
+        if out is not None and (out.dtype != torch.int32 or out.numel() != 1):
+            raise ValueError("group_contexts: out must be one int32 word")
         need = self.lib.glb_group_contexts_workspace(n)
         if self._ws is None or self._ws.numel() < need:
             self._ws = torch.empty(max(need, 1 << 16), dtype=torch.uint8, device=self.device)
-        group_of, rep, ng = self._i32(n), self._i32(n), self._i32(1)
+        group_of, rep, ng = self._i32(n), self._i32(n), self._i32(1) if out is None else out
         check(self.lib.glb_group_contexts(_ptr(tokens), _ptr(starts), _ptr(lengths), n, _ptr(hashes), _ptr(group_of),
                                           _ptr(rep), _ptr(ng), _ptr(self._ws), self._ws.numel(), self._stream()))
         return group_of, rep, ng
@@ -634,6 +650,44 @@
                                          self._stream()))
         return ids, am, pos, last
 
+    def packed_plan(self, tokens, starts, lengths, sel, n_sel, grp, groups, n_tail_rows, max_keys, pos_bound, out=None):
+        n_sel, n_tail_rows = int(n_sel), int(n_tail_rows)
+        G, n_pre = groups.lens_d.numel(), int(groups.n_rows)
+        for name, t, dt in (("tokens", tokens, torch.int32), ("starts", starts, torch.int64), ("lengths", lengths, torch.int32),
+                            ("sel", sel, torch.int32), ("grp", grp, torch.int32), ("groups.lens_d", groups.lens_d, torch.int32),
+                            ("groups.starts_d", groups.starts_d, torch.int32), ("groups.segments", groups.segments, torch.int32),
+                            ("groups.ids", groups.ids, torch.int64), ("groups.pos", groups.pos, torch.int64)):
+            if t.dtype != dt:
+                raise ValueError(f"packed_plan: {name} must be {dt}, not {t.dtype}")
+        self._check_dev(tokens, starts, lengths, sel, grp, groups.lens_d, groups.starts_d, groups.segments, groups.ids, groups.pos)
+        if n_sel < 1 or sel.numel() < n_sel or grp.numel() < n_sel or n_tail_rows < 0:
+            raise ValueError("packed_plan: sel and grp must hold n_sel >= 1 entries, n_tail_rows >= 0")
+        if starts.numel() != lengths.numel() or lengths.numel() < 1 or tokens.numel() < 1:
+            raise ValueError("packed_plan: starts and lengths must name the same contexts, of a batch with tokens")
+        if (G < 1 or groups.starts_d.numel() != G or groups.segments.numel() != 4 * G or groups.ids.numel() != n_pre
+                or groups.pos.numel() != n_pre):
+            raise ValueError("packed_plan: the prompt groups' arrays do not agree on their sizes")
+        M, dev = n_pre + n_tail_rows, self.device
+        if out is None:
+            out = (torch.empty((G + n_sel, 4), dtype=torch.int32, device=dev), torch.empty(M, dtype=torch.int64, device=dev),
+                   torch.empty(M, dtype=torch.int64, device=dev), torch.empty(n_sel, dtype=torch.int64, device=dev))
+        segments, ids, pos, last = out
+        self._check_dev(*out)
+        if (segments.dtype, ids.dtype, pos.dtype, last.dtype) != (torch.int32, torch.int64, torch.int64, torch.int64) or (
+                segments.numel(), ids.numel(), pos.numel(), last.numel()) != (4 * (G + n_sel), M, M, n_sel):
+            raise ValueError("packed_plan: out must be (int32 [G + n_sel, 4], int64 [M], int64 [M], int64 [n_sel])")
+        a = _lib.PackedPlanArgs()
+        a.struct_size = C.sizeof(_lib.PackedPlanArgs)
+        a.tokens, a.starts, a.lengths = tokens.data_ptr(), starts.data_ptr(), lengths.data_ptr()
+        a.n_tokens, a.n_ctx = tokens.numel(), lengths.numel()
+        a.sel, a.grp, a.n_sel = sel.data_ptr(), grp.data_ptr(), n_sel
+        a.group_lens, a.group_starts, a.group_segments = groups.lens_d.data_ptr(), groups.starts_d.data_ptr(), groups.segments.data_ptr()
+        a.group_ids, a.group_pos, a.n_groups, a.n_pre = groups.ids.data_ptr(), groups.pos.data_ptr(), G, n_pre
+        a.n_tail_rows, a.max_keys, a.pos_bound = n_tail_rows, int(max_keys), int(pos_bound)
+        a.out_segments, a.out_ids, a.out_pos, a.out_last_rows = segments.data_ptr(), ids.data_ptr(), pos.data_ptr(), last.data_ptr()
+        check(self.lib.glb_packed_plan(C.byref(a), self._stream()))
+        return segments, ids, pos, last
+
     def gather_kv_padded(self, slab_ptrs, slab_len, prefix_of, heads, head_dim, p_max, dtype):
         n_rows = prefix_of.numel()
         out = torch.empty((n_rows, heads, p_max, head_dim), dtype=dtype, device=self.device)
@@ -646,6 +700,17 @@
         n, ld = contexts.shape
         check(self.lib.glb_particles_advance(_ptr(contexts), ld, _ptr(lengths), _ptr(active), _ptr(log_weights),
                                              _ptr(logZ), _ptr(token), n, eos_id, max_len, _ptr(hashes), self._stream()))
+
+    def particles_advance2(self, contexts, lengths, active, log_weights, logZ, token, eos_id, max_len, hashes, prompt_len,
+                           hash_stub, max_tokens, head, to_global):
+        n, ld = check_advance2_args(contexts, lengths, active, log_weights, logZ, token, hashes, prompt_len, hash_stub, head)
+        self._check_dev(contexts, lengths, active, log_weights, logZ, token, hashes, prompt_len, hash_stub, head)
+        lengths_eff, hashes_eff, done = self._i32(n), torch.empty(n, dtype=torch.int64, device=self.device), self._i32(n)
+        check(self.lib.glb_particles_advance2(_ptr(contexts), ld, _ptr(lengths), _ptr(active), _ptr(log_weights), _ptr(logZ),
+                                              _ptr(token), n, eos_id, max_len, _ptr(hashes), _ptr(prompt_len), _ptr(hash_stub),
+                                              int(max_tokens), _ptr(lengths_eff), _ptr(hashes_eff), _ptr(done), _ptr(head),
+                                              int(bool(to_global)), self._stream()))
+        return lengths_eff, hashes_eff, done
 
     def normalize_weights(self, log_weights):
         n = log_weights.numel()
diff --git a/genlm-backend_amd/kv.py b/genlm-backend_amd/kv.py
--- a/genlm-backend_amd/kv.py
+++ b/genlm-backend_amd/kv.py
@@ -5,6 +5,8 @@
 import numpy as np
 import torch
 from transformers.cache_utils import Cache, CacheLayerMixin, DynamicCache
+
+from ._lib import PACKED_PLAN_MAX_SEL
 
 
 _ATTN_NAME = "glb"
@@ -622,15 +624,33 @@
     return bool(head_dim in (16, 32, 64, 128) and getattr(cfg, "num_hidden_layers", 0) > 0)
 
 
-def encode_packed(llm, batch, sel, n_sel, grp, groups, n_tail_rows, max_keys=PACKED_MAX_KEYS):
-    eng, dev = llm.engine, llm.device
-    tokens, starts, lengths = batch
+def encode_packed(llm, batch, sel, n_sel, grp, groups, n_tail_rows, max_keys=PACKED_MAX_KEYS, native_plan=True):
+    eng = llm.engine
     if not 1 <= max_keys <= PACKED_MAX_KEYS:
         raise ValueError(f"encode_packed serves contexts of up to {PACKED_MAX_KEYS} tokens")
     if n_sel < 1 or n_tail_rows < n_sel:
         raise ValueError("encode_packed: every context feeds at least one tail row")
     if not packed_supported(llm):
         raise RuntimeError("encode_packed: this model's attention is not served by glb_short_attention")
+    M = groups.n_rows + int(n_tail_rows)
+    max_pos = getattr(llm._body.config, "max_position_embeddings", None) or (1 << 30)
+    pos_bound = min(PACKED_MAX_KEYS, max_pos)
+    plan = getattr(eng, "packed_plan", None) if native_plan else None
+    if plan is not None and n_sel <= PACKED_PLAN_MAX_SEL:
+        segments, ids, pos, last = plan(*batch, sel, n_sel, grp, groups, n_tail_rows, max_keys, pos_bound)
+    else:
+        segments, ids, pos, last = _packed_plan_torch(batch, sel, n_sel, grp, groups, n_tail_rows, pos_bound)
+    pkv = PackedKV(eng, segments, M, max_keys, llm._body.config.num_hidden_layers)
+    out = llm._body(input_ids=ids.view(1, M), position_ids=pos.view(1, M), attention_mask=None, past_key_values=pkv, use_cache=True)
+    if pkv.served != len(pkv.layers):
+        raise RuntimeError(f"glb_short_attention_packed served {pkv.served} of {len(pkv.layers)} layers: an attention module "
+                           "bypassed the attention interface and attended across the packed contexts")
+    return PackedEncoding(out, last, M)
+
+
+def _packed_plan_torch(batch, sel, n_sel, grp, groups, n_tail_rows, pos_bound):
+    tokens, starts, lengths = batch
+    dev = lengths.device
     G, n_pre = len(groups.lens), groups.n_rows
     M = n_pre + int(n_tail_rows)
     sel_l, grp_l = sel[:n_sel].long(), grp[:n_sel].long().clamp(0, G - 1)
@@ -643,15 +663,9 @@
     u = torch.searchsorted(ends, r, right=True).clamp_(max=n_sel - 1)
     pos_t = (pre_len[u] + (r - (ends - tail)[u])).long()
     at = (starts[sel_l[u]] + pos_t).clamp_(0, tokens.numel() - 1)
-    ids = torch.cat([groups.ids, tokens[at].long()]).view(1, M)
-    max_pos = getattr(llm._body.config, "max_position_embeddings", None) or (1 << 30)
-    pos = torch.cat([groups.pos, pos_t.clamp_(0, min(PACKED_MAX_KEYS, max_pos) - 1)]).view(1, M)
-    pkv = PackedKV(eng, segments, M, max_keys, llm._body.config.num_hidden_layers)
-    out = llm._body(input_ids=ids, position_ids=pos, attention_mask=None, past_key_values=pkv, use_cache=True)
-    if pkv.served != len(pkv.layers):
-        raise RuntimeError(f"glb_short_attention_packed served {pkv.served} of {len(pkv.layers)} layers: an attention module "
-                           "bypassed the attention interface and attended across the packed contexts")
-    return PackedEncoding(out, (tail_start + tail - 1).long().clamp_(0, M - 1), M)
+    ids = torch.cat([groups.ids, tokens[at].long()])
+    pos = torch.cat([groups.pos, pos_t.clamp_(0, pos_bound - 1)])
+    return segments, ids, pos, (tail_start + tail - 1).long().clamp_(0, M - 1)
 
 
 class PrefixLRU:
diff --git a/genlm-backend_amd/sis.py b/genlm-backend_amd/sis.py
--- a/genlm-backend_amd/sis.py
+++ b/genlm-backend_amd/sis.py
@@ -135,7 +135,7 @@
     def __init__(self, llm, n_particles, prompt_ids, max_tokens, eos_id, seed=0, rng="philox", rank=0, world=1,
                  dist=None, use_prefix_kv=False, use_particle_kv=False, resample_ess=None, force_collectives=False,
                  share_kv=True, kv_rows=None, kv_in_place=0.75, kv_graph=True, particle_masks=None, migrate_kv=True,
-                 constraint=None, share_prompt_rows=True, proposal_temperature=None, proposal=None):
+                 constraint=None, share_prompt_rows=True, proposal_temperature=None, proposal=None, native_step_state=True):
         if constraint is not None and particle_masks is not None:
             raise ValueError("give particle_masks (the caller's bit rows) or constraint (masks made on the device), not both")
         self._propose = proposal_temperature is not None or proposal is not None
@@ -229,6 +229,9 @@
         self.rows_moved = 0
         self.resample_ess = resample_ess
         self.n_resamples = 0
+        self.native_step_state = bool(native_step_state)
+        self._head = torch.zeros(8, dtype=torch.int32, device=self.dev)
+        self._state_edits = 0
         self.sync_every = 1
         self.reset()
 
@@ -251,6 +254,7 @@
         if self.noise_src is not None:
             self.noise_src.reset()
         self._particle.reset()
+        self._touch_state()
         self.contexts = self._ctx0.clone()
         self.prompt_len = self._prompt_len0.clone()
         self._grp = self._grp0
@@ -277,8 +281,26 @@
 
     def _rehash(self):
         ctx_flat = self.contexts.view(-1)
+        self._touch_state()
         self.hashes = self.eng.hash_contexts(ctx_flat, self.starts, self.lengths)
         self._hash_stub = self.eng.hash_contexts(ctx_flat, self.starts, torch.ones_like(self.lengths))
+
+    def _touch_state(self):
+        self._state_edits += 1
+        self._state = None
+
+    def _state_stamp(self):
+        ts = (self.lengths, self.active, self.hashes, self.prompt_len)
+        return (self.t, self.n_resamples, self._state_edits) + tuple(id(x) for x in ts) + tuple(x._version for x in ts)
+
+    def _routes_state(self):
+        return (self.native_step_state and hasattr(self.eng, "particles_advance2") and not self.particle_kv
+                and not self._propose and not (self.collective and self.world > 1) and self.rng_mode != RNG_NOISE
+                and type(self)._finish_step is DeviceSIS._finish_step)
+
+    def _state_ok(self):
+        st = self.__dict__.get("_state")
+        return st[1] if st is not None and st[0] == self._state_stamp() else None
 
     @torch.no_grad()
     def _encode_into_slabs(self, rows):
@@ -348,10 +370,11 @@
         row_of = plan["logits_row"][group_of.long()]
         return self._finish_step(logits, row_of, U, n_active, n_global, time_kernel, l_max=1)
 
-    def _finish_step(self, logits, group_of, U, n_active, n_global, time_kernel, l_max):
+    def _finish_step(self, logits, group_of, U, n_active, n_global, time_kernel, l_max, route=False):
         eng, llm, N = self.eng, self.llm, self.N
         V = logits.shape[-1]
-        mask_id = ((self.lengths - self.prompt_len) >= self.max_tokens).to(torch.int32)
+        state = self._state_ok() if route else None
+        mask_id = state[2] if state is not None else ((self.lengths - self.prompt_len) >= self.max_tokens).to(torch.int32)
         if self._propose:
             return self._finish_proposed(logits, group_of, U, n_active, n_global, time_kernel, l_max, mask_id)
         source = self.constraint if self.constraint is not None else self._particle if self.particle_masks is not None else llm.masks
@@ -373,7 +396,7 @@
             self.outer_events.append((e0, e1))
         if self.rng_mode == RNG_NOISE:
             self.noise_src.prefetch()
-        return self._advance(logits, mask_id, logZ, tok, U, n_active, n_global, l_max)
+        return self._advance(logits, mask_id, logZ, tok, U, n_active, n_global, l_max, route)
 
     def _proposal_masks(self, logits, ids, by_row):
         key = "row_mask_id" if by_row else "mask_id"
@@ -403,16 +426,25 @@
             self.outer_events.append((e0, e1))
         return self._advance(logits, mask_id, dlogw, tok, U, n_active, n_global, l_max)
 
-    def _advance(self, logits, mask_id, logZ, tok, U, n_active, n_global, l_max):
+    def _advance(self, logits, mask_id, logZ, tok, U, n_active, n_global, l_max, route=False):
         eng = self.eng
         len_was = self.lengths.clone() if self.constraint is not None else None
         if self.constraint is not None and self.constraint.weighted:
             self.log_weights += self.constraint.forced_final_logw(self.states, (mask_id > 0) & (self.active > 0) & (tok == self.eos_id))
-        eng.particles_advance(self.contexts, self.lengths, self.active, self.log_weights, logZ, tok, self.eos_id,
-                              self.cap, hashes=self.hashes)
+        self._touch_state()
+        made = None
+        if route:
+            made = eng.particles_advance2(self.contexts, self.lengths, self.active, self.log_weights, logZ, tok, self.eos_id,
+                                          self.cap, self.hashes, self.prompt_len, self._hash_stub, self.max_tokens,
+                                          self._head, to_global=not self.collective)
+        else:
+            eng.particles_advance(self.contexts, self.lengths, self.active, self.log_weights, logZ, tok, self.eos_id,
+                                  self.cap, hashes=self.hashes)
         if self.constraint is not None:
             self.constraint.advance(self.states, self.contexts, len_was, self.lengths, out=self.states)
         self.t += 1
+        if made is not None:
+            self._state = (self._state_stamp(), made, (self.lengths, self.active, self.hashes, self.prompt_len))
         self.max_len_now = min(self.max_len_now + 1, self.cap)
         ft = self._fwd_tokens if self._fwd_tokens is not None else U * l_max
         self._fwd_tokens = None
@@ -439,6 +471,10 @@
         self._particle.update(rows, bit_rows)
 
     def _exchange(self):
+        if not self.collective and self._state_ok() is not None:
+            self.all_weights = self.log_weights
+            self._global_active = self._head[2]
+            return
         count = self.active.sum().to(torch.float32).view(1)
         if self.collective:
             N = self.N
@@ -469,6 +505,14 @@
         if self.particle_kv and self.t > 0:
             return self._step_particle_kv(time_kernel)
         ctx_flat = self.contexts.view(-1)
+        route = self._routes_state()
+        state = self._state_ok() if route else None
+        if state is not None:
+            lengths_eff, hashes_eff, _ = state
+            group_of, rep, ng = eng.group_contexts(ctx_flat, self.starts, lengths_eff, hashes=hashes_eff, out=self._head[0:1])
+            self._rep = rep
+            head = torch.cat([self._head[:2], self._global_active.view(1), eng.error_word()]).cpu()
+            return self._encode_and_finish(ctx_flat, lengths_eff, group_of, rep, head, time_kernel, route)
         lengths_eff = torch.where(self.active > 0, self.lengths, torch.ones_like(self.lengths))
         if self.particle_kv:
             head = torch.stack([self.active.sum().to(torch.int32), self._global_active, eng.error_word()[0]]).cpu()
@@ -482,6 +526,10 @@
         group_of, rep, ng = eng.group_contexts(ctx_flat, self.starts, lengths_eff, hashes=hashes_eff)
         self._rep = rep
         head = torch.stack([ng[0], self.active.sum().to(torch.int32), self._global_active, eng.error_word()[0]]).cpu()
+        return self._encode_and_finish(ctx_flat, lengths_eff, group_of, rep, head, time_kernel, route)
+
+    def _encode_and_finish(self, ctx_flat, lengths_eff, group_of, rep, head, time_kernel, route):
+        eng, llm = self.eng, self.llm
         U, n_active, n_global = int(head[0]), int(head[1]), int(head[2])
         eng.raise_if_failed(int(head[3]))
         base, prefixes = None, None
@@ -504,7 +552,7 @@
             other = self.proposal
             self._q_logits = other._lm_head(encode_ragged(other, (ctx_flat, self.starts, lengths_eff), rep, U, l_max).last_rows())
         self._noise_groups = None
-        return self._finish_step(logits, group_of, U, n_active, n_global, time_kernel, l_max)
+        return self._finish_step(logits, group_of, U, n_active, n_global, time_kernel, l_max, **({"route": True} if route else {}))
 
     def _packed_ready(self, U, n_active, l_max):
         if self._groups is None or self.t < 1 or n_active != self.N or l_max > PACKED_MAX_KEYS or self.prefixes is not None:
@@ -611,6 +659,7 @@
                     slots_d = torch.from_numpy(slots.astype(np.int64)).to(dev)
                     new_state[slots_d] = recv
                 moved = (take_d, send_cnt, slots_d, recv_cnt)
+        self._touch_state()
         self.contexts = new_state[:, :self.cap].contiguous()
         self.lengths, self.prompt_len, self.active = (new_state[:, self.cap + k].contiguous() for k in range(3))
         self.log_weights = (lse - float(np.log(n_total))).expand(N).contiguous()
@@ -733,6 +782,7 @@
         rows = torch.arange(N, device=dev)
         at = self.lengths.long().clamp_max(self.cap - 1)
         self.contexts[rows, at] = torch.where(keep, tok, self.contexts[rows, at])
+        self._touch_state()
         self.lengths = self.lengths + keep.to(torch.int32)
         self.active = torch.where(tok == -2, self.active, (keep & (self.lengths - self.prompt_len < self.max_tokens)).to(torch.int32))
         self.t += 1
diff --git a/include/glb.h b/include/glb.h
--- a/include/glb.h
+++ b/include/glb.h
@@ -122,6 +122,11 @@
 int glb_particles_advance(int32_t *contexts, int64_t ctx_ld, int32_t *lengths, int32_t *active,
                           float *log_weights, const float *logZ, const int32_t *token, int64_t n,
                           int32_t eos_id, int32_t max_len, uint64_t *ctx_hashes, void *hip_stream);
+int glb_particles_advance2(int32_t *contexts, int64_t ctx_ld, int32_t *lengths, int32_t *active, float *log_weights,
+                           const float *logZ, const int32_t *token, int64_t n, int32_t eos_id, int32_t max_len,
+                           uint64_t *ctx_hashes, const int32_t *prompt_len, const uint64_t *hash_stub, int32_t max_tokens,
+                           int32_t *out_lengths_eff, uint64_t *out_hashes_eff, int32_t *out_done, int32_t *head,
+                           int32_t to_global, void *hip_stream);
 
 int glb_normalize_weights(const float *log_weights, int64_t n, float *out_probs, float *out_stats,
                           void *hip_stream);
@@ -737,6 +742,26 @@
 int glb_score_rows(const glb_score_args *args, void *hip_stream);
 int glb_score_seq_sums(const float *values, int64_t n_rows, const int64_t *seq_start, int64_t n_seq, float *out, void *hip_stream);
 
+#define GLB_PACKED_PLAN_MAX_SEL (1 << 20)
+typedef struct {
+  uint32_t struct_size;
+  const int32_t *tokens;
+  const int64_t *starts;
+  const int32_t *lengths;
+  int64_t n_tokens, n_ctx;
+  const int32_t *sel, *grp;
+  int64_t n_sel;
+  const int32_t *group_lens, *group_starts, *group_segments;
+  const int64_t *group_ids, *group_pos;
+  int64_t n_groups, n_pre;
+  int64_t n_tail_rows;
+  int32_t max_keys;
+  int64_t pos_bound;
+  int32_t *out_segments;
+  int64_t *out_ids, *out_pos, *out_last_rows;
+} glb_packed_plan_args;
+int glb_packed_plan(const glb_packed_plan_args *args, void *hip_stream);
+
 void glb_philox4x32_10(const uint32_t ctr[4], const uint32_t key[2], uint32_t out[4]);
 
 #ifdef __cplusplus
```

Result: faster. 146,900, median of 5 (+3.0%).
